# yozoyugen/HAKAI-fem

Measured on AMD Instinct MI355X. Metric: M element-updates/sec (hex8, 8 Gauss pts) at 1/2/4/8 MI355X; % HBM roofline, higher is better.
Workload: dtype f64

## Files before the change

### hakai-fem_amd/csrc/hakai_capi.cpp

```cpp
#include <hip/hip_runtime.h>

#include <algorithm>
#include <cmath>
#include <cstdarg>
#include <cstdio>
#include <cstdlib>
#include <cstring>
#include <map>
#include <memory>
#include <string>
#include <vector>

#include "../../include/hakai_hip.h"
#include "hakai_conn_plan.hpp"
#include "hakai_elem_history.hpp"
#include "hakai_history.hpp"
#include "hakai_internal.hpp"
#include "hakai_kernels.hpp"
#include "hakai_loads.hpp"
#include "hakai_mass_scale.hpp"
#include "hakai_stable_dt.hpp"

using hk::DevMat;

namespace {
thread_local std::string g_err;
}

namespace hkc {

int fail(int code, const char* fmt, ...) {
    char buf[1024];
    va_list ap;
    va_start(ap, fmt);
    vsnprintf(buf, sizeof buf, fmt, ap);
    va_end(ap);
    g_err = buf;
    return code;
}

int hip_fail(hipError_t e, const char* what) {
    return fail(HAKAI_ERR_DEVICE, "%s: %s", what, hipGetErrorString(e));
}

}

using hkc::DevBuf;
using hkc::fail;
using hkc::hip_fail;
using hkc::QSrc;

namespace hkc {

static void free_model(hakai_ctx* c) {
    contact_destroy(c);
    loads_destroy(c);
    for (DevBuf<double>* b : {&c->d_coord, &c->d_u[0], &c->d_u[1], &c->d_mass, &c->d_stress, &c->d_strain, &c->d_eqps,
                              &c->d_yield, &c->d_triax, &c->d_fe, &c->d_qbuf})
        b->free();
    for (DevBuf<int>* b : {&c->d_conn, &c->d_flag, &c->d_mat, &c->d_inc_ptr, &c->d_inc, &c->d_inc_row, &c->d_inc8,
                           &c->d_del_step})
        b->free();
    c->d_mats.free();
    c->d_conn_rec.free();
    c->conn_P = 0;
    own_free(c);
    c->model_ok = false;
    c->state_ok = false;
}

int build_devmat(const hakai_material_t& in, DevMat& o) {
    std::memset(&o, 0, sizeof o);
    const double young = in.young, poisson = in.poisson;
    const double d1 = (1.0 - poisson), d2 = poisson, d3 = (1.0 - 2.0 * poisson) / 2.0;
    const double cc = young / (1.0 + poisson) / (1.0 - 2.0 * poisson);
    o.Dn = cc * d1;
    o.Do = cc * d2;
    o.Ds = cc * d3;
    o.G = young / 2. / (1.0 + poisson);
    o.density = in.density;
    if (in.n_plastic < 0 || in.n_plastic > hk::kMaxPlastic)
        return fail(HAKAI_ERR_ARG, "material: %d plastic rows (max %d)", in.n_plastic, hk::kMaxPlastic);
    if (in.n_ductile < 0 || in.n_ductile > hk::kMaxDuctile)
        return fail(HAKAI_ERR_ARG, "material: %d ductile rows (max %d)", in.n_ductile, hk::kMaxDuctile);
    if (in.n_plastic == 1)
        return fail(HAKAI_ERR_MODEL,
                    "material: a single *Plastic row gives an empty Hd; the reference raises BoundsError "
                    "(v2/HAKAI_j.jl:1267)");
    o.npp = in.n_plastic;
    o.nd = in.n_ductile;
    o.yield0 = in.n_plastic > 0 ? in.plastic[0] : 0.0;
    for (int r = 0; r < in.n_plastic; ++r) o.pl_eps[r] = in.plastic[2 * r + 1];
    for (int r = 0; r + 1 < in.n_plastic; ++r)
        o.Hd[r] = (in.plastic[2 * (r + 1)] - in.plastic[2 * r]) / (in.plastic[2 * (r + 1) + 1] - in.plastic[2 * r + 1]);
    for (int r = 0; r < in.n_ductile; ++r) {
        o.du_eps[r] = in.ductile[3 * r + 0];
        o.du_tri[r] = in.ductile[3 * r + 1];
    }
    double lo = 0.0, hi = 0.0;
    for (int r = 0; r < in.n_ductile; ++r) {
        lo = r == 0 ? o.du_eps[r] : std::min(lo, o.du_eps[r]);
        hi = r == 0 ? o.du_eps[r] : std::max(hi, o.du_eps[r]);
    }
    o.du_floor = in.n_ductile > 0 ? lo - (std::fabs(hi) + std::fabs(lo)) * 0x1p-40 : 0.0;
    if (!(o.du_floor == o.du_floor)) o.du_floor = -HUGE_VAL;
    o.du_skip = o.du_floor > 0.0 ? o.du_floor - o.du_floor * 0x1p-40 : -HUGE_VAL;
    return 0;
}

void pusai_table(double out[192]) {
    static const double delta[8][3] = {{-1.0, -1.0, -1.0}, {1.0, -1.0, -1.0}, {1.0, 1.0, -1.0}, {-1.0, 1.0, -1.0},
                                       {-1.0, -1.0, 1.0},  {1.0, -1.0, 1.0},  {1.0, 1.0, 1.0},  {-1.0, 1.0, 1.0}};
    const double g = 1.0 / std::sqrt(3.0);
    for (int k = 0; k < 8; ++k) {
        const double gzai = (k & 4) ? g : -g, eta = (k & 2) ? g : -g, tueta = (k & 1) ? g : -g;
        for (int i = 0; i < 8; ++i) {
            out[24 * k + i] = 1.0 / 8.0 * delta[i][0] * (1.0 + eta * delta[i][1]) * (1.0 + tueta * delta[i][2]);
            out[24 * k + 8 + i] = 1.0 / 8.0 * delta[i][1] * (1.0 + gzai * delta[i][0]) * (1.0 + tueta * delta[i][2]);
            out[24 * k + 16 + i] = 1.0 / 8.0 * delta[i][2] * (1.0 + gzai * delta[i][0]) * (1.0 + eta * delta[i][1]);
        }
    }
}

hipStream_t ctx_stream(hakai_ctx* c) { return c->stream; }
int ctx_device(hakai_ctx* c) { return c->device; }

}

static void prof_harvest(hakai_ctx* c) {
    if (c->ev_pending.empty()) return;
    (void)hipEventSynchronize(c->ev_pending.back().b);
    for (auto& p : c->ev_pending) {
        float ms = 0.f;
        if (hipEventElapsedTime(&ms, p.a, p.b) == hipSuccess) {
            c->k_ms[p.kernel] += ms;
            c->k_n[p.kernel] += 1;
        }
        c->ev_pool.push_back(p.a);
        c->ev_pool.push_back(p.b);
    }
    c->ev_pending.clear();
}

static hipEvent_t prof_event(hakai_ctx* c) {
    if (c->ev_pool.empty()) {
        if (c->ev_pending.size() >= 2048) prof_harvest(c);
        if (c->ev_pool.empty()) {
            hipEvent_t e;
            (void)hipEventCreate(&e);
            return e;
        }
    }
    hipEvent_t e = c->ev_pool.back();
    c->ev_pool.pop_back();
    return e;
}

namespace hkc {
void prof_begin(hakai_ctx* c, int kernel, EventPair* p) {
    p->kernel = -1;
    if (!c->prof || !((c->prof_mask >> kernel) & 1u)) return;
    p->kernel = kernel;
    p->a = prof_event(c);
    p->b = prof_event(c);
    (void)hipEventRecord(p->a, c->stream);
}
void prof_end(hakai_ctx* c, EventPair* p) {
    if (!c->prof || p->kernel < 0) return;
    (void)hipEventRecord(p->b, c->stream);
    c->ev_pending.push_back(*p);
}
}


namespace hkc {

hk::ElemArgs elem_args(const hakai_ctx* c, int cur) {
    hk::ElemArgs ea;
    std::memset(&ea, 0, sizeof ea);
    ea.coord = c->d_coord;
    ea.u = c->d_u[cur];
    ea.u_pre = c->d_u[1 - cur];
    ea.conn = c->d_conn;
    ea.flag = c->d_flag;
    ea.mat = c->d_mat;
    ea.mat_stride = c->nmat == 1 ? 0u : 4u;
    ea.mats = c->d_mats;
    ea.stress = c->d_stress;
    ea.strain = c->d_strain;
    for (int q = 0; q < 6; ++q) {
        ea.sc[q] = c->d_stress + q * c->ld;
        ea.ec[q] = c->d_strain + q * c->ld;
    }
    ea.eqps = c->d_eqps;
    ea.yield = c->d_yield;
    ea.triax = c->d_triax;
    ea.fe = c->d_fe;
    ea.vol = nullptr;
    ea.nE = c->nE;
    ea.nEp = c->nEp;
    ea.ld = c->ld;
    ea.del_step = c->d_del_step;
    ea.step_i = 0;
    ea.any_plastic = c->any_plastic ? 1 : 0;
    ea.pipe_blocks = pipe_grid(c) > 0 ? c->pipe_blocks : 0;
    ea.gp_nt = c->gp_nt;
    ea.nmat = c->nmat;
    ea.exact = c->elem_exact;
    ea.pusai = c->d_pusai;
    ea.poison = c->d_poison;
    return ea;
}

hk::NodalArgs nodal_args(const hakai_ctx* c, double d_time) {
    hk::NodalArgs na;
    na.u = c->d_u[c->sv.cur];
    na.u_pre_out = c->d_u[1 - c->sv.cur];
    na.mass = c->d_mass;
    na.inc_ptr = c->d_inc_ptr;
    na.inc = c->d_inc;
    na.inc8 = c->d_inc8;
    na.fe = c->d_fe;
    na.qbuf = c->sv.q == QSrc::Buf ? c->d_qbuf : nullptr;
    na.fext = nullptr;
    na.nN = c->nN;
    na.dt = d_time;
    na.bc_of_node = nullptr;
    const OwnSums o = c->sv.q == QSrc::Own ? own_sums(c) : OwnSums{nullptr, nullptr, nullptr, nullptr};
    na.own_q = o.q;
    na.own_rp = o.rp;
    na.own_rows = o.rows;
    na.own_ridx = o.ridx;
    na.poison = c->d_poison;
    return na;
}

hk::BCArgs bc_args(const hakai_ctx* c, double t, double d_time) {
    hk::BCArgs ba;
    ba.dof = c->bc.d_dof;
    ba.grp = c->bc.d_grp;
    ba.val = c->bc.d_val;
    ba.n = c->bc.n;
    ba.amp_n = c->bc.d_amp_n;
    ba.amp_off = c->bc.d_amp_off;
    ba.amp_t = c->bc.d_amp_t;
    ba.amp_v = c->bc.d_amp_v;
    ba.out = c->d_u[1 - c->sv.cur];
    ba.ct = t * d_time;
    ba.t_rd = c->gr.trd;
    ba.dt = d_time;
    ba.poison = c->d_poison;
    return ba;
}

}

static int fe_download_qe(hakai_ctx* c, double* Qe) {
    HIPCHK(hipMemcpyAsync(Qe, c->d_fe, 24 * (size_t)c->nE * sizeof(double), hipMemcpyDeviceToHost, c->stream));
    HIPCHK(hipStreamSynchronize(c->stream));
    return 0;
}

static int fe_upload_qe(hakai_ctx* c, const double* Qe) {
    HIPCHK(hipMemcpyAsync(c->d_fe, Qe, 24 * (size_t)c->nE * sizeof(double), hipMemcpyHostToDevice, c->stream));
    HIPCHK(hipStreamSynchronize(c->stream));
    return 0;
}

static int fe_upload_incidence(hakai_ctx* c) {
    std::vector<int> inc(c->h_inc0.size());
    for (size_t j = 0; j < inc.size(); ++j) inc[j] = 24 * (c->h_inc0[j] >> 3) + 3 * (c->h_inc0[j] & 7);
    if (!inc.empty())
        HIPCHK(hipMemcpyAsync(c->d_inc, inc.data(), inc.size() * sizeof(int), hipMemcpyHostToDevice, c->stream));
    if (c->d_inc8) {
        std::vector<int> inc8(8 * (size_t)c->nN, (int)(24 * c->nEp));
        for (long long n = 0; n < c->nN; ++n)
            for (int j = c->h_ptr[n]; j < c->h_ptr[n + 1]; ++j) inc8[8 * n + (j - c->h_ptr[n])] = inc[j];
        HIPCHK(hipMemcpyAsync(c->d_inc8, inc8.data(), inc8.size() * sizeof(int), hipMemcpyHostToDevice, c->stream));
    }
    HIPCHK(hipStreamSynchronize(c->stream));
    return 0;
}

extern "C" {

int hakai_abi_version(void) { return HAKAI_ABI_VERSION; }
const char* hakai_last_error(void) { return g_err.c_str(); }

int hakai_device_count(int* n) {
    if (!n) return fail(HAKAI_ERR_ARG, "null");
    int cnt = 0;
    if (hipGetDeviceCount(&cnt) != hipSuccess) cnt = 0;
    *n = cnt;
    return 0;
}

int hakai_create(hakai_ctx** out, int device) {
    if (!out) return fail(HAKAI_ERR_ARG, "null ctx pointer");
    *out = nullptr;
    int cnt = 0;
    if (hipGetDeviceCount(&cnt) != hipSuccess || cnt <= 0)
        return fail(HAKAI_ERR_DEVICE, "no HIP device visible: the HAKAI MI355X path has no CPU fallback");
    if (device < 0 || device >= cnt) return fail(HAKAI_ERR_ARG, "device %d out of range (%d visible)", device, cnt);
    HIPCHK(hipSetDevice(device));
    hipDeviceProp_t prop;
    HIPCHK(hipGetDeviceProperties(&prop, device));
    if (std::strncmp(prop.gcnArchName, "gfx950", 6) != 0)
        return fail(HAKAI_ERR_DEVICE, "device %d is %s; libhakai_hip is built for gfx950 only", device,
                    prop.gcnArchName);
    struct Drop {
        void operator()(hakai_ctx* p) const {
            if (p->stream) (void)hipStreamDestroy(p->stream);
            delete p;
        }
    };
    std::unique_ptr<hakai_ctx, Drop> c(new hakai_ctx());
    c->device = device;
    if (const char* v = std::getenv("HAKAI_PIPE_BLOCKS")) c->pipe_blocks = std::atoi(v);
    if (const char* v = std::getenv("HAKAI_GRAPH")) {
        const int g = std::atoi(v);
        c->graph = (g >= 0 && g <= 1024 && !(g & 1)) ? g : 0;
    }
    hipError_t e = hipStreamCreateWithFlags(&c->stream, hipStreamNonBlocking);
    if (e != hipSuccess) return hip_fail(e, "hipStreamCreate");
    if (c->d_negjac.alloc(1) != hipSuccess || c->d_pusai.alloc(192) != hipSuccess ||
        c->d_poison.alloc(2) != hipSuccess || hipMemset(c->d_poison, 0, 2 * sizeof(int)) != hipSuccess)
        return fail(HAKAI_ERR_DEVICE, "hipMalloc for context bookkeeping failed");
    {
        double pus[192];
        hkc::pusai_table(pus);
        bool odd = true;
        for (int k = 0; k < 8; ++k)
            for (int i = 0; i < 8; ++i) {
                const double* p = pus + 24 * k;
                odd = odd && p[i] == -p[i ^ 1] && p[8 + i] == -p[8 + (i ^ 3)] && p[16 + i] == -p[16 + (i ^ 4)];
            }
        e = odd ? hipMemcpy(c->d_pusai, pus, sizeof pus, hipMemcpyHostToDevice) : hipErrorInvalidValue;
        if (e != hipSuccess) return hip_fail(e, "hipMemcpy (Pusai table)");
    }
    if (const char* v = std::getenv("HAKAI_ELEM_EXACT")) c->elem_exact = std::atoi(v) ? 1 : 0;
    if (const char* v = std::getenv("HAKAI_OWN_ASSEMBLY")) c->own.assembly = std::atoi(v) ? 1 : 0;
    *out = c.release();
    return 0;
}

int hakai_destroy(hakai_ctx* c) {
    if (!c) return 0;
    (void)hipSetDevice(c->device);
    (void)hipStreamSynchronize(c->stream);
    prof_harvest(c);
    hkc::graph_free(c);
    hkc::history_destroy(c);
    hkc::elem_history_destroy(c);
    hkc::stable_dt_destroy(c);
    hkc::mass_scale_destroy(c);
    hkc::comm_destroy(c);
    hkc::free_model(c);
    for (auto e : c->ev_pool) (void)hipEventDestroy(e);
    (void)hipStreamDestroy(c->stream);
    delete c;
    return 0;
}

int hakai_upload_model(hakai_ctx* c, int64_t nNode, const double* coordmat, int64_t nElement,
                       const int64_t* elementmat, const int64_t* element_material, int32_t nMat,
                       const hakai_material_t* mats, const double* diag_M) {
    if (c) hkc::graph_invalidate(c);
    if (!c) return fail(HAKAI_ERR_ARG, "null ctx");
    if (nNode <= 0 || nElement < 0 || !coordmat || (nElement > 0 && (!elementmat || !element_material)) || nMat <= 0 ||
        !mats || !diag_M)
        return fail(HAKAI_ERR_ARG, "upload_model: bad arguments");
    if (26 * (nElement + 32) + 8 >= (int64_t)INT32_MAX || nNode >= (int64_t)INT32_MAX)
        return fail(HAKAI_ERR_ARG, "upload_model: mesh too large for int32 indexing on one rank");
    if (192 * (nElement + 32) >= (int64_t)1 << 32)
        return fail(HAKAI_ERR_ARG, "upload_model: %lld elements exceed one context's 32-bit element-kernel offsets "
                    "(max %lld); split the mesh over ranks", (long long)nElement, (long long)(((int64_t)1 << 32) / 192 - 32));
    if (24 * (nNode + 1) >= (int64_t)1 << 32)
        return fail(HAKAI_ERR_ARG, "upload_model: %lld nodes exceed one context's 32-bit element-kernel offsets "
                    "(max %lld); split the mesh over ranks", (long long)nNode, (long long)(((int64_t)1 << 32) / 24 - 1));
    HIPCHK(hipSetDevice(c->device));
    (void)hipStreamSynchronize(c->stream);
    hkc::history_destroy(c);
    hkc::elem_history_destroy(c);
    hkc::stable_dt_destroy(c);
    hkc::mass_scale_destroy(c);
    hkc::free_model(c);
    c->bc = {};
    const long long nN = nNode, nE = nElement;
    const long long nEp = ((nE + 31) / 32) * 32;
    std::vector<int> conn((size_t)(8 * nEp), 0), mat((size_t)nEp, 0);
    for (long long e = 0; e < nE; ++e) {
        for (int i = 0; i < 8; ++i) {
            const int64_t n = elementmat[8 * e + i];
            if (n < 1 || n > nN) return fail(HAKAI_ERR_ARG, "elementmat[%d,%lld] = %lld out of 1..%lld", i + 1, e + 1, (long long)n, nN);
            conn[8 * e + i] = (int)(n - 1);
        }
        const int64_t m = element_material[e];
        if (m < 1 || m > nMat) return fail(HAKAI_ERR_ARG, "element_material[%lld] = %lld out of 1..%d", e + 1, (long long)m, nMat);
        mat[e] = (int)(m - 1);
    }
    std::vector<double> mass((size_t)nN);
    for (long long n = 0; n < nN; ++n) {
        const double m0 = diag_M[3 * n], m1 = diag_M[3 * n + 1], m2 = diag_M[3 * n + 2];
        if (!(m0 == m1 && m1 == m2))
            return fail(HAKAI_ERR_ARG, "diag_M: node %lld has different masses per dof", n + 1);
        mass[n] = m0;
    }
    c->h_mats.assign((size_t)nMat, DevMat());
    c->nmat = nMat;
    c->has_ductile = false;
    for (int i = 0; i < nMat; ++i) {
        int r = hkc::build_devmat(mats[i], c->h_mats[i]);
        if (r) return r;
    }
    c->any_plastic = false;
    for (long long e = 0; e < nE; ++e) {
        if (c->h_mats[mat[e]].nd > 0) c->has_ductile = true;
        if (c->h_mats[mat[e]].npp > 0) c->any_plastic = true;
    }
    std::vector<int> ptr((size_t)nN + 1, 0), inc((size_t)(8 * nE));
    for (long long j = 0; j < 8 * nE; ++j) ptr[conn[j] + 1]++;
    for (long long n = 0; n < nN; ++n) ptr[n + 1] += ptr[n];
    {
        std::vector<int> fill(ptr.begin(), ptr.end() - 1);
        for (long long j = 0; j < 8 * nE; ++j) inc[fill[conn[j]]++] = (int)j;
    }
    int maxinc = 0;
    for (long long n = 0; n < nN; ++n) maxinc = std::max(maxinc, ptr[n + 1] - ptr[n]);
    c->nN = nN;
    c->nE = nE;
    c->nEp = nEp;
    c->ld = 8 * nEp;
    const size_t ld = (size_t)c->ld;
    HIPCHK(c->d_coord.alloc(3 * (size_t)nN));
    HIPCHK(c->d_u[0].alloc(3 * (size_t)nN));
    HIPCHK(c->d_u[1].alloc(3 * (size_t)nN));
    HIPCHK(c->d_mass.alloc((size_t)nN));
    HIPCHK(c->d_conn.alloc(8 * (size_t)nEp));
    HIPCHK(c->d_flag.alloc((size_t)nEp));
    HIPCHK(c->d_mat.alloc((size_t)nEp));
    HIPCHK(c->d_del_step.alloc((size_t)nEp + 2));
    HIPCHK(c->d_mats.alloc((size_t)nMat));
    HIPCHK(c->d_stress.alloc(6 * ld));
    HIPCHK(c->d_strain.alloc(6 * ld));
    HIPCHK(c->d_eqps.alloc(ld));
    HIPCHK(c->d_yield.alloc(ld));
    HIPCHK(c->d_triax.alloc(ld));
    c->fe_len = 26 * nEp + 8;
    HIPCHK(c->d_fe.alloc((size_t)c->fe_len));
    HIPCHK(c->d_inc_ptr.alloc((size_t)nN + 1));
    HIPCHK(c->d_inc.alloc(8 * (size_t)nE));
    HIPCHK(c->d_inc_row.alloc(8 * (size_t)nE));
    HIPCHK(c->d_qbuf.alloc(3 * (size_t)nN));
    hipStream_t s = c->stream;
    HIPCHK(hipMemcpyAsync(c->d_coord, coordmat, 3 * nN * sizeof(double), hipMemcpyHostToDevice, s));
    HIPCHK(hipMemcpyAsync(c->d_mass, mass.data(), nN * sizeof(double), hipMemcpyHostToDevice, s));
    if (nE) {
        HIPCHK(hipMemcpyAsync(c->d_conn, conn.data(), 8 * nEp * sizeof(int), hipMemcpyHostToDevice, s));
        HIPCHK(hipMemcpyAsync(c->d_mat, mat.data(), nEp * sizeof(int), hipMemcpyHostToDevice, s));
        HIPCHK(hipMemcpyAsync(c->d_inc_row, inc.data(), 8 * nE * sizeof(int), hipMemcpyHostToDevice, s));
    }
    {
        hk::ConnPlan cp;
        if (nE && hk::conn_plan(conn.data(), nEp, cp)) {
            std::vector<unsigned> rp(cp.rec);
            rp.insert(rp.end(), cp.pat.begin(), cp.pat.end());
            HIPCHK(c->d_conn_rec.upload(rp, s));
            HIPCHK(hipStreamSynchronize(s));
            c->conn_P = cp.P;
            c->conn_bits = cp.base_bits;
            c->conn_bytes = cp.bytes;
        }
    }
    HIPCHK(hipMemcpyAsync(c->d_mats, c->h_mats.data(), nMat * sizeof(DevMat), hipMemcpyHostToDevice, s));
    HIPCHK(hipMemcpyAsync(c->d_inc_ptr, ptr.data(), (nN + 1) * sizeof(int), hipMemcpyHostToDevice, s));
    if (maxinc <= 8) HIPCHK(c->d_inc8.alloc(8 * (size_t)nN));
    HIPCHK(hipStreamSynchronize(s));
    c->max_inc = maxinc;
    c->h_ptr = ptr;
    c->h_inc0 = inc;
    {
        int r = fe_upload_incidence(c);
        if (r) return r;
    }
    c->h_coord.assign(coordmat, coordmat + 3 * nN);
    c->h_conn.assign(conn.begin(), conn.begin() + 8 * nE);
    c->h_mat.assign(mat.begin(), mat.begin() + nE);
    c->h_young.resize((size_t)nMat);
    for (int i = 0; i < nMat; ++i) c->h_young[i] = mats[i].young;
    c->h_poisson.resize((size_t)nMat);
    for (int i = 0; i < nMat; ++i) c->h_poisson[i] = mats[i].poisson;
    c->model_ok = true;
    c->state_ok = false;
    return hakai_reset_state(c, 0, nullptr, nullptr, 1.0);
}

int hakai_set_bc(hakai_ctx* c, const hakai_bc_t* bc) {
    if (c) hkc::graph_invalidate(c);
    if (!c || !bc) return fail(HAKAI_ERR_ARG, "null");
    if (!c->model_ok) return fail(HAKAI_ERR_STATE, "set_bc before upload_model");
    HIPCHK(hipSetDevice(c->device));
    (void)hipStreamSynchronize(c->stream);
    c->bc = {};
    const int G = bc->n_groups;
    if (G <= 0) return hkc::history_bc_changed(c);
    std::map<long long, std::pair<int, double>> last;
    for (int g = 0; g < G; ++g) {
        if (bc->amp_n[g] == 1)
            return fail(HAKAI_ERR_MODEL, "BC group %d: one-point amplitude, the reference raises BoundsError (:598)", g + 1);
        for (int64_t en = bc->entry_off[g]; en < bc->entry_off[g + 1]; ++en)
            for (int64_t d = bc->dof_off[en]; d < bc->dof_off[en + 1]; ++d) {
                const int64_t dof = bc->dofs[d];
                if (dof < 1 || dof > 3 * c->nN) return fail(HAKAI_ERR_ARG, "BC dof %lld out of range", (long long)dof);
                last[dof - 1] = std::make_pair(g, bc->entry_value[en]);
            }
    }
    std::vector<int> dof, grp;
    std::vector<double> val;
    for (auto& kv : last) {
        dof.push_back((int)kv.first);
        grp.push_back(kv.second.first);
        val.push_back(kv.second.second);
    }
    std::vector<int> amp_n(G), amp_off(G);
    long long n_amp = 0;
    for (int g = 0; g < G; ++g) {
        amp_n[g] = bc->amp_n[g];
        amp_off[g] = (int)bc->amp_off[g];
        n_amp = std::max<long long>(n_amp, bc->amp_off[g] + bc->amp_n[g]);
    }
    c->bc.n = (int)dof.size();
    HIPCHK(c->bc.d_dof.alloc(dof.size()));
    HIPCHK(c->bc.d_grp.alloc(grp.size()));
    HIPCHK(c->bc.d_val.alloc(val.size()));
    HIPCHK(c->bc.d_amp_n.alloc((size_t)G));
    HIPCHK(c->bc.d_amp_off.alloc((size_t)G));
    HIPCHK(c->bc.d_amp_t.alloc((size_t)n_amp));
    HIPCHK(c->bc.d_amp_v.alloc((size_t)n_amp));
    hipStream_t s = c->stream;
    if (!dof.empty()) {
        HIPCHK(hipMemcpyAsync(c->bc.d_dof, dof.data(), dof.size() * sizeof(int), hipMemcpyHostToDevice, s));
        HIPCHK(hipMemcpyAsync(c->bc.d_grp, grp.data(), grp.size() * sizeof(int), hipMemcpyHostToDevice, s));
        HIPCHK(hipMemcpyAsync(c->bc.d_val, val.data(), val.size() * sizeof(double), hipMemcpyHostToDevice, s));
    }
    HIPCHK(hipMemcpyAsync(c->bc.d_amp_n, amp_n.data(), G * sizeof(int), hipMemcpyHostToDevice, s));
    HIPCHK(hipMemcpyAsync(c->bc.d_amp_off, amp_off.data(), G * sizeof(int), hipMemcpyHostToDevice, s));
    if (n_amp) {
        HIPCHK(hipMemcpyAsync(c->bc.d_amp_t, bc->amp_time, n_amp * sizeof(double), hipMemcpyHostToDevice, s));
        HIPCHK(hipMemcpyAsync(c->bc.d_amp_v, bc->amp_value, n_amp * sizeof(double), hipMemcpyHostToDevice, s));
    }
    if (!dof.empty()) {
        std::vector<int> of((size_t)c->nN, -1);
        for (size_t i = dof.size(); i-- > 0;) of[(size_t)dof[i] / 3] = (int)i;
        HIPCHK(c->bc.d_of_node.alloc(of.size()));
        HIPCHK(hipMemcpyAsync(c->bc.d_of_node, of.data(), of.size() * sizeof(int), hipMemcpyHostToDevice, s));
    }
    HIPCHK(hipStreamSynchronize(s));
    return hkc::history_bc_changed(c);
}

int hakai_reset_state(hakai_ctx* c, int64_t n_ic, const int64_t* ic_dofs, const double* ic_values, double d_time) {
    if (c) hkc::graph_invalidate(c);
    if (!c) return fail(HAKAI_ERR_ARG, "null");
    if (!c->model_ok) return fail(HAKAI_ERR_STATE, "reset_state before upload_model");
    HIPCHK(hipSetDevice(c->device));
    hipStream_t s = c->stream;
    const size_t fn = 3 * (size_t)c->nN;
    c->sv.restart(false);
    HIPCHK(hipMemsetAsync(c->d_u[0], 0, fn * sizeof(double), s));
    HIPCHK(hipMemsetAsync(c->d_u[1], 0, fn * sizeof(double), s));
    HIPCHK(hipMemsetAsync(c->d_fe, 0, (size_t)c->fe_len * sizeof(double), s));
    HIPCHK(hipMemsetAsync(c->d_del_step, 0, ((size_t)c->nEp + 2) * sizeof(int), s));
    HIPCHK(hk::launch_reset_gp(c->d_stress, c->d_strain, c->d_eqps, c->d_yield, c->d_triax, c->d_flag, c->d_mat,
                               c->d_mats, c->nE, c->nEp, c->ld, s));
    c->h_velo0.assign(fn, 0.0);
    HIPCHK(hipMemsetAsync(c->d_poison, 0, 2 * sizeof(int), s));
    hkc::comm_reset(c);
    if (n_ic > 0) {
        if (!ic_dofs || !ic_values) return fail(HAKAI_ERR_ARG, "reset_state: null IC arrays");
        std::vector<double> dpre(fn, 0.0);
        for (int64_t j = 0; j < n_ic; ++j) {
            const int64_t d = ic_dofs[j];
            if (d < 1 || d > (int64_t)fn) return fail(HAKAI_ERR_ARG, "IC dof %lld out of range", (long long)d);
            dpre[d - 1] = -ic_values[j] * d_time;
            c->h_velo0[d - 1] = ic_values[j];
        }
        HIPCHK(hipMemcpyAsync(c->d_u[1 - c->sv.cur], dpre.data(), fn * sizeof(double), hipMemcpyHostToDevice, s));
        HIPCHK(hipStreamSynchronize(s));
    }
    c->state_ok = true;
    if (int r = hkc::contact_state_reset(c, c->h_velo0.data())) return r;
    if (int r = hkc::history_restart(c)) return r;
    if (int r = hkc::elem_history_restart(c)) return r;
    HIPCHK(hipStreamSynchronize(s));
    return 0;
}

int hakai_upload_state(hakai_ctx* c, const hakai_state_t* st) {
    if (c) hkc::graph_invalidate(c);
    if (!c || !st) return fail(HAKAI_ERR_ARG, "null");
    if (!c->model_ok) return fail(HAKAI_ERR_STATE, "upload_state before upload_model");
    HIPCHK(hipSetDevice(c->device));
    if (c->sv.q == QSrc::Own && !c->sv.fe_ok && !st->Q && !st->Qe) {
        bool dels = false;
        for (long long e = 0; st->element_flag && e < c->nE && !dels; ++e) dels = st->element_flag[e] == 0;
        if (dels || c->comm)
            return fail(HAKAI_ERR_STATE, "upload_state: the last element step's forces exist only as owner-computed "
                        "node sums (a contact overflow skipped the call's last step); upload Q (from "
                        "hakai_download_state) or Qe with this state");
        if (int r = hkc::own_materialize(c)) return r;
    }
    c->sv.restart(true);
    hipStream_t s = c->stream;
    const size_t fn = 3 * (size_t)c->nN, nGP = 8 * (size_t)c->nE;
    if (st->disp) HIPCHK(hipMemcpyAsync(c->d_u[c->sv.cur], st->disp, fn * sizeof(double), hipMemcpyHostToDevice, s));
    if (st->disp_pre)
        HIPCHK(hipMemcpyAsync(c->d_u[1 - c->sv.cur], st->disp_pre, fn * sizeof(double), hipMemcpyHostToDevice, s));
    if (st->velo) c->h_velo0.assign(st->velo, st->velo + fn);
    if (st->Q) {
        HIPCHK(hipMemcpyAsync(c->d_qbuf, st->Q, fn * sizeof(double), hipMemcpyHostToDevice, s));
        c->sv.q_uploaded();
    }
    if (st->integ_stress || st->integ_strain) {
        DevBuf<double> tmp;
        HIPCHK(tmp.alloc(6 * nGP));
        if (st->integ_stress) {
            HIPCHK(hipMemcpyAsync(tmp, st->integ_stress, 6 * nGP * sizeof(double), hipMemcpyHostToDevice, s));
            HIPCHK(hk::launch_aos_to_soa6(tmp, c->d_stress, (long long)nGP, c->ld, s));
        }
        if (st->integ_strain) {
            HIPCHK(hipMemcpyAsync(tmp, st->integ_strain, 6 * nGP * sizeof(double), hipMemcpyHostToDevice, s));
            HIPCHK(hk::launch_aos_to_soa6(tmp, c->d_strain, (long long)nGP, c->ld, s));
        }
        HIPCHK(hipStreamSynchronize(s));
    }
    if (st->integ_yield_stress)
        HIPCHK(hipMemcpyAsync(c->d_yield, st->integ_yield_stress, nGP * sizeof(double), hipMemcpyHostToDevice, s));
    if (st->integ_eq_plastic_strain)
        HIPCHK(hipMemcpyAsync(c->d_eqps, st->integ_eq_plastic_strain, nGP * sizeof(double), hipMemcpyHostToDevice, s));
    if (st->integ_triax_stress)
        HIPCHK(hipMemcpyAsync(c->d_triax, st->integ_triax_stress, nGP * sizeof(double), hipMemcpyHostToDevice, s));
    if (st->element_flag) {
        std::vector<int> f((size_t)c->nE);
        for (long long e = 0; e < c->nE; ++e) f[e] = st->element_flag[e] != 0 ? 1 : 0;
        HIPCHK(hipMemcpyAsync(c->d_flag, f.data(), c->nE * sizeof(int), hipMemcpyHostToDevice, s));
        std::vector<int> ds((size_t)c->nE);
        for (long long e = 0; e < c->nE; ++e) ds[e] = f[e] ? 0 : -1;
        HIPCHK(hipMemcpyAsync(c->d_del_step, ds.data(), c->nE * sizeof(int), hipMemcpyHostToDevice, s));
        HIPCHK(hipMemsetAsync(c->d_del_step + c->nEp, 0, 2 * sizeof(int), s));
        HIPCHK(hipStreamSynchronize(s));
        bool any = false;
        for (long long e = 0; e < c->nE; ++e) any |= !f[e];
        if (any && !st->Qe) {
            std::vector<double> qe(24 * (size_t)c->nE);
            int r = fe_download_qe(c, qe.data());
            if (r) return r;
            for (long long e = 0; e < c->nE; ++e)
                if (!f[e]) std::fill(qe.begin() + 24 * e, qe.begin() + 24 * (e + 1), 0.0);
            if ((r = fe_upload_qe(c, qe.data()))) return r;
        }
    }
    if (st->Qe) {
        int r = fe_upload_qe(c, st->Qe);
        if (r) return r;
    }
    HIPCHK(hipMemsetAsync(c->d_poison, 0, 2 * sizeof(int), s));
    HIPCHK(hipStreamSynchronize(s));
    hkc::comm_reset(c);
    c->state_ok = true;
    if (int r = hkc::history_restart(c)) return r;
    if (int r = hkc::elem_history_restart(c)) return r;
    if (c->contact) {
        if (int r = hkc::contact_state_reset(c, c->h_velo0.empty() ? nullptr : c->h_velo0.data())) return r;
        HIPCHK(hipStreamSynchronize(s));
    }
    return 0;
}

int hakai_download_state(hakai_ctx* c, hakai_state_t* st) {
    if (!c || !st) return fail(HAKAI_ERR_ARG, "null");
    if (!c->state_ok) return fail(HAKAI_ERR_STATE, "download_state without state");
    if (st->Qe && !c->sv.fe_ok)
        return fail(HAKAI_ERR_STATE, "download_state: Qe is not available after a call whose last steps a contact "
                    "overflow skipped (owner-computed assembly keeps node sums only); Q is -- or step once more");
    if (st->integ_triax_stress && !c->sv.triax_ok)
        return fail(HAKAI_ERR_STATE, "download_state: integ_triax_stress is not available after a call whose last "
                    "steps a contact overflow skipped (it is stored on a call's last step); step once more");
    HIPCHK(hipSetDevice(c->device));
    hipStream_t s = c->stream;
    const size_t fn = 3 * (size_t)c->nN, nGP = 8 * (size_t)c->nE;
    HIPCHK(hipStreamSynchronize(s));
    if (st->disp) HIPCHK(hipMemcpyAsync(st->disp, c->d_u[c->sv.cur], fn * sizeof(double), hipMemcpyDeviceToHost, s));
    if (st->disp_pre)
        HIPCHK(hipMemcpyAsync(st->disp_pre, c->d_u[1 - c->sv.cur], fn * sizeof(double), hipMemcpyDeviceToHost, s));
    if (st->velo) {
        if (c->sv.steps_done == 0) {
            std::memcpy(st->velo, c->h_velo0.data(), fn * sizeof(double));
        } else {
            std::vector<double> a(fn), b(fn);
            HIPCHK(hipMemcpyAsync(a.data(), c->d_u[c->sv.cur], fn * sizeof(double), hipMemcpyDeviceToHost, s));
            HIPCHK(hipMemcpyAsync(b.data(), c->d_u[1 - c->sv.cur], fn * sizeof(double), hipMemcpyDeviceToHost, s));
            HIPCHK(hipStreamSynchronize(s));
            for (size_t i = 0; i < fn; ++i) {
                const double dd = a[i] - b[i];
                st->velo[i] = dd / c->last_dt;
            }
        }
    }
    if (st->Q) {
        if (c->sv.q == QSrc::Buf) {
            HIPCHK(hipMemcpyAsync(st->Q, c->d_qbuf, fn * sizeof(double), hipMemcpyDeviceToHost, s));
        } else {
            DevBuf<double> tmp;
            HIPCHK(tmp.alloc(fn));
            if (c->sv.q == QSrc::Own) {
                const hkc::OwnSums o = hkc::own_sums(c);
                HIPCHK(hk::launch_own_q(o.q, o.rp, o.ridx, o.rows, tmp, c->nN, s));
            } else
                HIPCHK(hk::launch_gather_q(c->d_inc_ptr, c->d_inc, c->d_fe, tmp, c->nN, s));
            HIPCHK(hipMemcpyAsync(st->Q, tmp, fn * sizeof(double), hipMemcpyDeviceToHost, s));
            HIPCHK(hipStreamSynchronize(s));
        }
    }
    if (st->integ_stress || st->integ_strain) {
        DevBuf<double> tmp;
        HIPCHK(tmp.alloc(6 * nGP));
        if (st->integ_stress) {
            HIPCHK(hk::launch_soa_to_aos6(c->d_stress, tmp, (long long)nGP, c->ld, s));
            HIPCHK(hipMemcpyAsync(st->integ_stress, tmp, 6 * nGP * sizeof(double), hipMemcpyDeviceToHost, s));
            HIPCHK(hipStreamSynchronize(s));
        }
        if (st->integ_strain) {
            HIPCHK(hk::launch_soa_to_aos6(c->d_strain, tmp, (long long)nGP, c->ld, s));
            HIPCHK(hipMemcpyAsync(st->integ_strain, tmp, 6 * nGP * sizeof(double), hipMemcpyDeviceToHost, s));
            HIPCHK(hipStreamSynchronize(s));
        }
    }
    if (st->integ_yield_stress)
        HIPCHK(hipMemcpyAsync(st->integ_yield_stress, c->d_yield, nGP * sizeof(double), hipMemcpyDeviceToHost, s));
    if (st->integ_eq_plastic_strain)
        HIPCHK(hipMemcpyAsync(st->integ_eq_plastic_strain, c->d_eqps, nGP * sizeof(double), hipMemcpyDeviceToHost, s));
    if (st->integ_triax_stress)
        HIPCHK(hipMemcpyAsync(st->integ_triax_stress, c->d_triax, nGP * sizeof(double), hipMemcpyDeviceToHost, s));
    if (st->element_flag) {
        std::vector<int> f((size_t)c->nE);
        HIPCHK(hipMemcpyAsync(f.data(), c->d_flag, c->nE * sizeof(int), hipMemcpyDeviceToHost, s));
        HIPCHK(hipStreamSynchronize(s));
        for (long long e = 0; e < c->nE; ++e) st->element_flag[e] = (f[e] == 1) ? 1 : 0;
    }
    if (st->Qe) {
        int r = fe_download_qe(c, st->Qe);
        if (r) return r;
    }
    HIPCHK(hipStreamSynchronize(s));
    return 0;
}

int hakai_stat(hakai_ctx* c, const char* key, int64_t* value) {
    if (!c || !key || !value) return fail(HAKAI_ERR_ARG, "null");
    if (!std::strcmp(key, "graph_steps")) *value = c->graph_steps;
    else if (!std::strcmp(key, "device_buffers")) *value = hkc::g_dev_live.load();
    else if (!std::strcmp(key, "exchange_retries")) *value = c->exchange_retries;
    else if (!std::strncmp(key, "own_", 4) || !std::strncmp(key, "conn_", 5)) return hkc::own_stat(c, key, value);
    else return fail(HAKAI_ERR_ARG, "unknown stat '%s'", key);
    return 0;
}

int hakai_sync(hakai_ctx* c) {
    if (!c) return fail(HAKAI_ERR_ARG, "null");
    HIPCHK(hipSetDevice(c->device));
    HIPCHK(hipStreamSynchronize(c->stream));
    return 0;
}

int hakai_deleted(hakai_ctx* c, int64_t* n_deleted, int64_t* log, int64_t cap) {
    if (!c) return fail(HAKAI_ERR_ARG, "null");
    if (!c->model_ok) return fail(HAKAI_ERR_STATE, "deleted before upload_model");
    HIPCHK(hipSetDevice(c->device));
    std::vector<int> ds((size_t)c->nE);
    if (c->nE) HIPCHK(hipMemcpyAsync(ds.data(), c->d_del_step, c->nE * sizeof(int), hipMemcpyDeviceToHost, c->stream));
    HIPCHK(hipStreamSynchronize(c->stream));
    std::vector<std::pair<long long, long long>> v;
    for (long long e = 0; e < c->nE; ++e)
        if (ds[e] > 0) v.push_back(std::make_pair((long long)ds[e], e + 1 + c->elem_offset));
    std::sort(v.begin(), v.end());
    if (n_deleted) *n_deleted = (int64_t)v.size();
    if (log)
        for (long long i = 0; i < (long long)v.size() && i < cap; ++i) {
            log[2 * i] = v[i].first;
            log[2 * i + 1] = v[i].second;
        }
    return 0;
}

int hakai_set_tuning(hakai_ctx* c, const char* key, int64_t value) {
    if (c) hkc::graph_invalidate(c);
    if (!c || !key) return fail(HAKAI_ERR_ARG, "set_tuning: null");
    if (!std::strcmp(key, "elem_pipe_blocks")) {
        if (value < 0 || value > 65536) return fail(HAKAI_ERR_ARG, "elem_pipe_blocks out of range");
        c->pipe_blocks = (int)value;
        return 0;
    }
    if (!std::strcmp(key, "elem_gp_nt")) {
        if (value != 0 && value != 1) return fail(HAKAI_ERR_ARG, "elem_gp_nt must be 0 or 1");
        c->gp_nt = (int)value;
        return 0;
    }
    if (!std::strcmp(key, "fuse_bc")) {
        if (value < 0 || value > 2) return fail(HAKAI_ERR_ARG, "fuse_bc must be 0, 1 or 2 (any mesh size)");
        c->fuse_bc = (int)value;
        return 0;
    }
    if (!std::strcmp(key, "elem_pipe_min")) {
        if (value < 0 || value > 1024) return fail(HAKAI_ERR_ARG, "elem_pipe_min out of range");
        c->pipe_min = (int)value;
        return 0;
    }
    if (!std::strcmp(key, "elem_exact")) {
        if (value != 0 && value != 1) return fail(HAKAI_ERR_ARG, "elem_exact must be 0 or 1");
        if (c->elem_exact != (int)value)
            if (int r = hkc::own_tuning(c, key, value)) return r;
        c->elem_exact = (int)value;
        return 0;
    }
    if (!std::strcmp(key, "group_serial")) {
        if (value < 0 || value > 2) return fail(HAKAI_ERR_ARG, "group_serial must be 0, 1 or 2");
        c->group_serial = (int)value;
        return 0;
    }
    if (!std::strcmp(key, "nodal_padded")) {
        if (!value) {
            c->d_inc8.free();
            return 0;
        }
        return c->d_inc8 ? 0 : fail(HAKAI_ERR_STATE, "padded incidence table unavailable (>8 incidences)");
    }
    if (!std::strncmp(key, "own_", 4)) return hkc::own_tuning(c, key, value);
    if (!std::strcmp(key, "conn_templates")) {
        if (value != 0 && value != 1) return fail(HAKAI_ERR_ARG, "conn_templates must be 0 or 1");
        c->conn_templates = (int)value;
        return 0;
    }
    if (!std::strcmp(key, "graph")) {
        if (value < 0 || value > 1024 || (value & 1)) return fail(HAKAI_ERR_ARG, "graph must be 0 or an even step count <= 1024");
        c->graph = (int)value;
        return 0;
    }
    if (!std::strcmp(key, "history_one_block")) {
        if (value < -1 || value > 1) return fail(HAKAI_ERR_ARG, "history_one_block must be -1 (by size), 0 or 1");
        c->hist_one_block = (int)value;
        return 0;
    }
    if (!std::strcmp(key, "elem_history_one_block")) {
        if (value < -1 || value > 1) return fail(HAKAI_ERR_ARG, "elem_history_one_block must be -1 (by size), 0 or 1");
        c->ehist_one_block = (int)value;
        return 0;
    }
    if (!std::strncmp(key, "contact_", 8)) {
        HIPCHK(hipSetDevice(c->device));
        return hkc::contact_tuning(c, key, value);
    }
    return fail(HAKAI_ERR_ARG, "unknown tuning key '%s'", key);
}

int hakai_set_element_offset(hakai_ctx* c, int64_t element_offset) {
    if (c) hkc::graph_invalidate(c);
    if (!c || element_offset < 0) return fail(HAKAI_ERR_ARG, "set_element_offset: bad args");
    c->elem_offset = element_offset;
    return 0;
}

int hakai_negative_jacobians(hakai_ctx* c, int64_t* n) {
    if (!c || !n) return fail(HAKAI_ERR_ARG, "null");
    if (!c->state_ok) return fail(HAKAI_ERR_STATE, "negative_jacobians without state");
    HIPCHK(hipSetDevice(c->device));
    HIPCHK(hipMemsetAsync(c->d_negjac, 0, sizeof(unsigned long long), c->stream));
    HIPCHK(hk::launch_negjac(hkc::elem_args(c, c->sv.cur), c->d_negjac, c->stream));
    unsigned long long v = 0;
    HIPCHK(hipMemcpyAsync(&v, c->d_negjac, sizeof v, hipMemcpyDeviceToHost, c->stream));
    HIPCHK(hipStreamSynchronize(c->stream));
    *n = (int64_t)v;
    return 0;
}

int hakai_node_stress_strain(hakai_ctx* c, double* node_stress, double* node_strain, double* node_eqps,
                             double* node_mises, double* node_triax) {
    if (!c) return fail(HAKAI_ERR_ARG, "null");
    if (!c->state_ok) return fail(HAKAI_ERR_STATE, "node_stress_strain without state");
    HIPCHK(hipSetDevice(c->device));
    hipStream_t s = c->stream;
    const size_t nN = (size_t)c->nN;
    DevBuf<double> ns, nn, ne, nm, nt;
    HIPCHK(ns.alloc(6 * nN));
    HIPCHK(nn.alloc(6 * nN));
    HIPCHK(ne.alloc(nN));
    HIPCHK(nm.alloc(nN));
    HIPCHK(nt.alloc(nN));
    HIPCHK(hk::launch_node_average(c->d_inc_ptr, c->d_inc_row, c->d_stress, c->d_strain, c->d_eqps, c->d_triax, c->ld,
                                   c->nN, ns, nn, ne, nm, nt, s));
    if (node_stress) HIPCHK(hipMemcpyAsync(node_stress, ns, 6 * nN * sizeof(double), hipMemcpyDeviceToHost, s));
    if (node_strain) HIPCHK(hipMemcpyAsync(node_strain, nn, 6 * nN * sizeof(double), hipMemcpyDeviceToHost, s));
    if (node_eqps) HIPCHK(hipMemcpyAsync(node_eqps, ne, nN * sizeof(double), hipMemcpyDeviceToHost, s));
    if (node_mises) HIPCHK(hipMemcpyAsync(node_mises, nm, nN * sizeof(double), hipMemcpyDeviceToHost, s));
    if (node_triax) HIPCHK(hipMemcpyAsync(node_triax, nt, nN * sizeof(double), hipMemcpyDeviceToHost, s));
    HIPCHK(hipStreamSynchronize(s));
    return 0;
}

int hakai_profile_enable(hakai_ctx* c, int on) { return hakai_profile_mask(c, on ? (1u << HAKAI_K_COUNT) - 1 : 0u); }

int hakai_profile_mask(hakai_ctx* c, uint32_t mask) {
    if (c) hkc::graph_invalidate(c);
    if (!c) return fail(HAKAI_ERR_ARG, "null");
    if (!mask) prof_harvest(c);
    c->prof = mask != 0;
    c->prof_mask = mask;
    for (int k = 0; k < HAKAI_K_COUNT; ++k) {
        c->k_ms[k] = 0;
        c->k_n[k] = 0;
    }
    return 0;
}

int hakai_profile_read(hakai_ctx* c, int kernel, double* total_ms, int64_t* launches) {
    if (!c || kernel < 0 || kernel >= HAKAI_K_COUNT) return fail(HAKAI_ERR_ARG, "bad profile query");
    (void)hipSetDevice(c->device);
    prof_harvest(c);
    if (total_ms) *total_ms = c->k_ms[kernel];
    if (launches) *launches = c->k_n[kernel];
    return 0;
}

int hakai_stress_hexa(int device, int64_t nNode, int64_t nElement, double* Qe, double* integ_stress,
                      double* integ_strain, double* integ_yield_stress, double* integ_eq_plastic_strain,
                      const double* position, const double* d_disp, const int64_t* elementmat,
                      const int64_t* element_flag, int32_t integ_num, int32_t nMat, const hakai_material_t* mats,
                      const int64_t* element_material, double* elementVolume) {
    if (integ_num != 8) return fail(HAKAI_ERR_ARG, "integ_num must be 8 (v2/HAKAI_j.jl:177)");
    if (!Qe || !integ_stress || !integ_strain || !integ_yield_stress || !integ_eq_plastic_strain || !position ||
        !d_disp || !element_flag)
        return fail(HAKAI_ERR_ARG, "stress_hexa: null array");
    hakai_ctx* c = nullptr;
    int r = hakai_create(&c, device);
    if (r) return r;
    struct Guard {
        hakai_ctx* c;
        ~Guard() { hakai_destroy(c); }
    } guard{c};
    std::vector<double> ones(3 * (size_t)nNode, 1.0);
    r = hakai_upload_model(c, nNode, position, nElement, elementmat, element_material, nMat, mats, ones.data());
    if (r) return r;
    std::vector<double> zero(3 * (size_t)nNode, 0.0), mdu(3 * (size_t)nNode);
    for (size_t i = 0; i < mdu.size(); ++i) mdu[i] = -d_disp[i];
    hakai_state_t st;
    std::memset(&st, 0, sizeof st);
    st.disp = zero.data();
    st.disp_pre = mdu.data();
    st.integ_stress = integ_stress;
    st.integ_strain = integ_strain;
    st.integ_yield_stress = integ_yield_stress;
    st.integ_eq_plastic_strain = integ_eq_plastic_strain;
    st.element_flag = const_cast<int64_t*>(element_flag);
    r = hakai_upload_state(c, &st);
    if (r) return r;
    hipStream_t s = c->stream;
    DevBuf<double> d_vol;
    HIPCHK(d_vol.alloc((size_t)c->nEp));
    HIPCHK(hipMemsetAsync(c->d_fe, 0, 24 * (size_t)nElement * sizeof(double), s));
    hk::ElemArgs ea = hkc::elem_args(c, c->sv.cur);
    ea.vol = d_vol;
    ea.pipe_blocks = 0;
    HIPCHK(hk::launch_element(ea, false, false, s));
    std::vector<double> fe(24 * (size_t)nElement), vol((size_t)nElement);
    HIPCHK(hipMemcpyAsync(fe.data(), c->d_fe, fe.size() * sizeof(double), hipMemcpyDeviceToHost, s));
    HIPCHK(hipMemcpyAsync(vol.data(), d_vol, vol.size() * sizeof(double), hipMemcpyDeviceToHost, s));
    HIPCHK(hipStreamSynchronize(s));
    hakai_state_t out;
    std::memset(&out, 0, sizeof out);
    out.integ_stress = integ_stress;
    out.integ_strain = integ_strain;
    out.integ_yield_stress = integ_yield_stress;
    out.integ_eq_plastic_strain = integ_eq_plastic_strain;
    r = hakai_download_state(c, &out);
    if (r) return r;
    for (int64_t e = 0; e < nElement; ++e) {
        if (element_flag[e] == 0) continue;
        for (int j = 0; j < 24; ++j) Qe[24 * e + j] += fe[24 * e + j];
        if (elementVolume) elementVolume[e] = vol[e];
    }
    return 0;
}

int hakai_triax_stress(int device, int64_t nGP, const double* integ_stress, double* integ_triax_stress) {
    if (nGP < 0 || (nGP > 0 && (!integ_stress || !integ_triax_stress))) return fail(HAKAI_ERR_ARG, "triax: bad args");
    int cnt = 0;
    if (hipGetDeviceCount(&cnt) != hipSuccess || cnt <= device || device < 0)
        return fail(HAKAI_ERR_DEVICE, "no HIP device %d: no CPU fallback", device);
    HIPCHK(hipSetDevice(device));
    if (nGP == 0) return 0;
    DevBuf<double> st, tx;
    HIPCHK(st.alloc(6 * (size_t)nGP));
    HIPCHK(tx.alloc((size_t)nGP));
    HIPCHK(hipMemcpy(st, integ_stress, 6 * nGP * sizeof(double), hipMemcpyHostToDevice));
    HIPCHK(hk::launch_triax_aos(st, tx, nGP, 0));
    HIPCHK(hipMemcpy(integ_triax_stress, tx, nGP * sizeof(double), hipMemcpyDeviceToHost));
    return 0;
}

}

namespace hkc {
long long ctx_nN(hakai_ctx* c) { return c->nN; }
}
```

### hakai-fem_amd/csrc/hakai_elem_fused.hpp

```cpp
#pragma once
#include "hakai_elem_io.hpp"
#include "hakai_exact_math.hpp"

namespace hk {


template <bool DO_DELETE, bool STORE_TRIAX, bool ANY_PLASTIC, bool WITH_VOL, int NT = 0, bool OWN = false>
__device__ __forceinline__ void elem_step(const ElemArgs& a, const DevMat* __restrict__ mats, long long e, int k,
                                          double* nd8, const ElemIn& in, double* sfe = nullptr) {
    const DevMat* M = mats + in.mt;
    const bool active = in.fl == 1;
    const int npp = M->npp;
    const int nd = DO_DELETE ? M->nd : 0;
    double eqp = in.eqp, ys = in.ys;

    nd8[6 * k + 0] = in.x[0];
    nd8[6 * k + 1] = in.x[1];
    nd8[6 * k + 2] = in.x[2];
    nd8[6 * k + 3] = in.du[0];
    nd8[6 * k + 4] = in.du[1];
    nd8[6 * k + 5] = in.du[2];
    wave_lds_fence();

    const double g = 1.0 / __builtin_sqrt(3.0);
    const double hp = 1.0 + g, hm = 1.0 - g;
    int nodej[8];
#pragma unroll
    for (int j = 0; j < 8; ++j) nodej[j] = 6 * ref_of_sign(j ^ k);
#define HK_MG(j, b) ((((j) >> (b)) & 1) ? hm : hp)
#define HK_SG(j, b) ((((j) >> (b)) & 1) ? 1.0 : -1.0)
#define HK_D0(j) (HK_SG(j, 2) * (1.0 / 8.0 * HK_MG(j, 1) * HK_MG(j, 0)))
#define HK_D1(j) (HK_SG(j, 1) * (1.0 / 8.0 * HK_MG(j, 2) * HK_MG(j, 0)))
#define HK_D2(j) (HK_SG(j, 0) * (1.0 / 8.0 * HK_MG(j, 2) * HK_MG(j, 1)))
    double J[3][3] = {{0., 0., 0.}, {0., 0., 0.}, {0., 0., 0.}};
#pragma unroll
    for (int j = 0; j < 8; ++j) {
        const double* X = nd8 + nodej[j];
        const double X0 = X[0], X1 = X[1], X2 = X[2];
        const double p0 = HK_D0(j), p1 = HK_D1(j), p2 = HK_D2(j);
        J[0][0] += p0 * X0; J[0][1] += p0 * X1; J[0][2] += p0 * X2;
        J[1][0] += p1 * X0; J[1][1] += p1 * X1; J[1][2] += p1 * X2;
        J[2][0] += p2 * X0; J[2][1] += p2 * X1; J[2][2] += p2 * X2;
    }
    const double c11 = J[1][1] * J[2][2] - J[1][2] * J[2][1];
    const double c21 = J[1][2] * J[2][0] - J[1][0] * J[2][2];
    const double c31 = J[1][0] * J[2][1] - J[1][1] * J[2][0];
    const double dett = J[0][0] * c11 + J[0][1] * c21 + J[0][2] * c31;
    const double det = (__builtin_popcount(k) & 1) ? -dett : dett;
    const double rd = 1.0 / dett;
    const double i11 = c11 * rd, i21 = c21 * rd, i31 = c31 * rd;
    const double i12 = (J[0][2] * J[2][1] - J[0][1] * J[2][2]) * rd;
    const double i22 = (J[0][0] * J[2][2] - J[0][2] * J[2][0]) * rd;
    const double i32 = (J[0][1] * J[2][0] - J[0][0] * J[2][1]) * rd;
    const double i13 = (J[0][1] * J[1][2] - J[0][2] * J[1][1]) * rd;
    const double i23 = (J[0][2] * J[1][0] - J[0][0] * J[1][2]) * rd;
    const double i33 = (J[0][0] * J[1][1] - J[0][1] * J[1][0]) * rd;
    double P[8][3];
#pragma unroll
    for (int j = 0; j < 8; ++j) {
        const double p0 = HK_D0(j), p1 = HK_D1(j), p2 = HK_D2(j);
        P[j][0] = i11 * p0 + i12 * p1 + i13 * p2;
        P[j][1] = i21 * p0 + i22 * p1 + i23 * p2;
        P[j][2] = i31 * p0 + i32 * p1 + i33 * p2;
    }
#undef HK_D0
#undef HK_D1
#undef HK_D2
#undef HK_SG
#undef HK_MG

    const double V = allreduce8(fabs(det));
    double wbar[3];
    {
        double v[8][3];
#pragma unroll
        for (int j = 0; j < 8; ++j)
#pragma unroll
            for (int c = 0; c < 3; ++c) v[j][c] = det * P[j][c];
        reduce_scatter8_rel(v, wbar);
    }
    const double r3V = 1.0 / (3.0 * V);
    const double bb0 = wbar[0] * r3V, bb1 = wbar[1] * r3V, bb2 = wbar[2] * r3V;
    const double* dn = nd8 + nodej[0] + 3;
    const double sdot = allreduce8(bb0 * dn[0] + bb1 * dn[1] + bb2 * dn[2]);

    double Gm[3][3] = {{0., 0., 0.}, {0., 0., 0.}, {0., 0., 0.}};
#pragma unroll
    for (int j = 0; j < 8; ++j) {
        const double* D = nd8 + nodej[j] + 3;
        const double d0 = D[0], d1 = D[1], d2 = D[2];
#pragma unroll
        for (int c = 0; c < 3; ++c) {
            Gm[0][c] += d0 * P[j][c];
            Gm[1][c] += d1 * P[j][c];
            Gm[2][c] += d2 * P[j][c];
        }
    }
    constexpr double kThird = 1.0 / 3.0;
    const double vol = sdot - (Gm[0][0] + Gm[1][1] + Gm[2][2]) * kThird;
    double de[6];
    de[0] = Gm[0][0] + vol;
    de[1] = Gm[1][1] + vol;
    de[2] = Gm[2][2] + vol;
    de[3] = Gm[0][1] + Gm[1][0];
    de[4] = Gm[1][2] + Gm[2][1];
    de[5] = Gm[0][2] + Gm[2][0];

    const double Dn = M->Dn, Do = M->Do, Ds = M->Ds;
    double fin[6];
    fin[0] = in.sig[0] + (Dn * de[0] + Do * (de[1] + de[2]));
    fin[1] = in.sig[1] + (Dn * de[1] + Do * (de[0] + de[2]));
    fin[2] = in.sig[2] + (Dn * de[2] + Do * (de[0] + de[1]));
    fin[3] = in.sig[3] + Ds * de[3];
    fin[4] = in.sig[4] + Ds * de[4];
    fin[5] = in.sig[5] + Ds * de[5];
    const double mean = (fin[0] + fin[1] + fin[2]) * kThird;
    double dv0 = fin[0] - mean, dv1 = fin[1] - mean, dv2 = fin[2] - mean;
    const double q =
        sqrt(1.5 * (dv0 * dv0 + dv1 * dv1 + dv2 * dv2 + 2.0 * (fin[3] * fin[3] + fin[4] * fin[4] + fin[5] * fin[5])));
    double sc = 1.0;
    if (ANY_PLASTIC && npp > 0 && q > ys) {
        const int p = plastic_segment(M->pl_eps, npp, eqp);
        const double H = M->Hd[p];
        const double dep = (q - ys) / (3.0 * M->G + H);
        sc = (ys + H * dep) / q;
        dv0 *= sc;
        dv1 *= sc;
        dv2 *= sc;
        fin[0] = dv0 + mean;
        fin[1] = dv1 + mean;
        fin[2] = dv2 + mean;
        fin[3] *= sc;
        fin[4] *= sc;
        fin[5] *= sc;
        eqp += dep;
        ys += H * dep;
    }
    double eps[6];
#pragma unroll
    for (int c = 0; c < 6; ++c) eps[c] = in.eps[c] + de[c];

    const double oeq = q * sc;
    double tri = STORE_TRIAX ? ((oeq < 1e-10) ? 0.0 : mean / oeq) : 0.0;
    bool kill = false;
    if (DO_DELETE && nd > 0 && __builtin_amdgcn_ballot_w64(eqp >= M->du_skip) != 0) {
        const double v_e = allreduce8(eqp) * 0.125;
        if (!STORE_TRIAX) tri = (oeq < 1e-10) ? 0.0 : mean / oeq;
        const double t_e = allreduce8(tri) * 0.125;
        if (!(t_e < 0.0) && v_e >= M->du_floor)
            kill = active && v_e >= ductile_fr(M->du_eps, M->du_tri, nd, t_e);
    }

    double fk[3];
    {
        const double w00 = det * dv0, w11 = det * dv1, w22 = det * dv2;
        const double w01 = det * fin[3], w12 = det * fin[4], w02 = det * fin[5];
        double v[8][3];
#pragma unroll
        for (int i = 0; i < 8; ++i) {
            const double px = P[i][0], py = P[i][1], pz = P[i][2];
            v[i][0] = w00 * px + w01 * py + w02 * pz;
            v[i][1] = w01 * px + w11 * py + w12 * pz;
            v[i][2] = w02 * px + w12 * py + w22 * pz;
        }
        reduce_scatter8_rel(v, fk);
    }
    const double S = allreduce8(det * (3.0 * mean));
    fk[0] += S * bb0;
    fk[1] += S * bb1;
    fk[2] += S * bb2;
    if (WITH_VOL) a.vol[e] = V;
    elem_writeback<DO_DELETE, STORE_TRIAX, ANY_PLASTIC, NT, false, OWN>(a, e, k, in, active, kill, fk, fin, eps, eqp,
                                                                         ys, tri, sfe);
}

}
```

### hakai-fem_amd/csrc/hakai_element.hip

```cpp
#include <hip/hip_runtime.h>

#include <algorithm>
#include <type_traits>

#include "hakai_elem_exact.hpp"
#include "hakai_elem_fused.hpp"
#include "hakai_elem_io.hpp"
#include "hakai_kernels.hpp"
#include "hakai_own_pass.hpp"

namespace hk {

template <bool DO_DELETE, bool STORE_TRIAX, bool WITH_VOL, bool EXACT>
__global__ __launch_bounds__(kBlock, 2) void k_element(ElemArgs a) {
    __shared__ __attribute__((aligned(16))) double s_nd[kEPB * kLdsStride];
    __shared__ __attribute__((aligned(16))) double s_xb[EXACT ? kEPB * kXbStride : 1];
    __shared__ __attribute__((aligned(16))) double s_pus[EXACT ? 8 * kPusStride : 1];
    const long long vb = xcd_remap(blockIdx.x, gridDim.x);
    if (poisoned(a.poison)) return;
    graph_step(a);
    const int k = threadIdx.x & 7;
    const int grp = threadIdx.x >> 3;
    if (EXACT) {
        stage_pusai(a, s_pus);
        __syncthreads();
    }
    const long long e = vb * kEPB + grp;
    ElemIn in;
    load_stage_a<EXACT>(a, e, k, in);
    if (EXACT) {
        load_node_raw(a, in);
        load_gp<true>(a, e, k, in);
    } else {
        load_stage_b<true>(a, e, k, in);
    }
#ifdef HK_DIAG_PHASE
    PhaseClock pc;
#endif
    if (EXACT)
        elem_step_exact<DO_DELETE, STORE_TRIAX, true, WITH_VOL>(a, a.mats, e, k, s_nd + grp * kLdsStride,
                                                                s_xb + grp * kXbStride, s_pus, in, nullptr HK_PH_PASS);
    else
        elem_step<DO_DELETE, STORE_TRIAX, true, WITH_VOL>(a, a.mats, e, k, s_nd + grp * kLdsStride, in);
}

#ifdef HK_DIAG_WAVE
constexpr int kDiagWaves = 8192, kDiagWords = 8;
__device__ unsigned long long g_diag[kDiagWaves * kDiagWords];
#endif

template <bool DO_DELETE, bool STORE_TRIAX, bool ANY_PLASTIC, bool LDS_MATS, int NT, bool EXACT, int OS = 0,
          bool TPL = false, bool CT = false>
__global__ __launch_bounds__(kBlock, 2) void k_element_pipe(ElemArgs a) {
    constexpr bool OWN = OS > 0;
    constexpr int kOwnFe = OS * kEPB * kFeStride;
    __shared__ __attribute__((aligned(16))) double s_nd[kEPB * kLdsStride];
    __shared__ __attribute__((aligned(16))) double s_fe[OWN ? 2 * kOwnFe : 1];
    extern __shared__ __attribute__((aligned(16))) double s_dyn[];
    double* s_part = s_dyn;
    DevMat* s_mats = reinterpret_cast<DevMat*>(s_dyn + (OWN ? 3 * a.own_slots : 0));
    __shared__ __attribute__((aligned(16))) double s_xb[EXACT ? kEPB * kXbStride : 1];
    __shared__ __attribute__((aligned(16))) double s_pus[EXACT ? 8 * kPusStride : 1];
    if (poisoned(a.poison)) return;
    graph_step(a);
    const int k = threadIdx.x & 7;
    const int grp = threadIdx.x >> 3;
    if (LDS_MATS) {
        const int words = a.nmat * (int)(sizeof(DevMat) / sizeof(double));
        const double* src = reinterpret_cast<const double*>(a.mats);
        double* dst = reinterpret_cast<double*>(s_mats);
        for (int w = threadIdx.x; w < words; w += kBlock) dst[w] = src[w];
    }
    if (EXACT) stage_pusai(a, s_pus);
    if (LDS_MATS || EXACT) __syncthreads();
    const DevMat* mats = LDS_MATS ? s_mats : a.mats;
    double* nd8 = s_nd + grp * kLdsStride;
    double* xb = s_xb + (EXACT ? grp * kXbStride : 0);
    const long long nb = a.nEp / kEPB;
    long long first, stride, count;
    if (OWN) {
        first = a.own_bstart[blockIdx.x];
        stride = 1;
        count = a.own_bstart[blockIdx.x + 1] - first;
    } else if (gridDim.x % 8 != 0) {
        first = (long long)blockIdx.x * nb / gridDim.x;
        stride = 1;
        count = ((long long)blockIdx.x + 1) * nb / gridDim.x - first;
    } else {
        const long long x = blockIdx.x & 7, j = blockIdx.x >> 3, per = gridDim.x >> 3;
        const long long r0 = x * nb / 8, r1 = (x + 1) * nb / 8;
        first = r0 + j;
        stride = per;
        count = first < r1 ? (r1 - first + per - 1) / per : 0;
    }
    if (count <= 0) return;
    auto pos_of = [&](long long i) { return first + (i < count ? i : count - 1) * stride; };
    auto vb_of = [&](long long i) { return OWN ? (long long)a.own_seq[pos_of(i)] : pos_of(i); };
    auto elem_of = [&](long long i) { return vb_of(i) * kEPB + grp; };

#ifdef HK_DIAG_WAVE
    PassClock dg;
    const long long dg_t0 = clock64();
#endif
#ifdef HK_DIAG_PHASE
    PhaseClock pc;
#endif
    ElemIn cur, nxt;
    int4 ent_cur = {0, 0, 0, 0}, ent_nxt = {0, 0, 0, 0};
    load_stage_a<EXACT, CT>(a, elem_of(0), k, cur);
    load_stage_a<EXACT, CT>(a, elem_of(1), k, nxt);
    static_assert(!(CT && EXACT), "connectivity templates: fused kernel only");
    int rec_nn = 0;
    if (CT) {
        const int r0 = conn_rec(a, elem_of(0)), r1 = conn_rec(a, elem_of(1));
        cur.n = conn_node(a, r0, conn_off(a, r0, k));
        nxt.n = conn_node(a, r1, conn_off(a, r1, k));
        rec_nn = conn_rec(a, elem_of(2));
    }
    if (!EXACT) load_stage_b<ANY_PLASTIC, NT>(a, elem_of(0), k, cur);
    constexpr int S = OS > 0 ? OS : 1;
    auto sb_of = [&](long long i) { return pos_of((i < count ? i : count - 1) / S * S); };
    int4 hdr_cur = {0, 0, 0, 0}, hdr_nxt = {0, 0, 0, 0}, hdr_nn = {0, 0, 0, 0};
    if (OWN && TPL) {
        hdr_cur = own_hdr_load(a, sb_of(0));
        hdr_nxt = own_hdr_load(a, sb_of(1));
        ent_cur = own_load_tpl(a, hdr_cur);
    } else if (OWN) {
        ent_cur = own_load(a, sb_of(0));
    }
    for (long long i = 0; i < count; ++i) {
        ElemIn nn;
        load_stage_a<EXACT, CT>(a, elem_of(i + 2), k, nn);
        int off = 0;
        if (CT) {
            nn.n = rec_nn;
            rec_nn = conn_rec(a, elem_of(i + 3));
            off = conn_off(a, nn.n, k);
        }
        if (OWN && TPL) hdr_nn = own_hdr_load(a, sb_of(i + 2));
        if (!EXACT) load_stage_b<ANY_PLASTIC, NT>(a, elem_of(i + 1), k, nxt);
        if (OWN) ent_nxt = TPL ? own_load_tpl(a, hdr_nxt) : own_load(a, sb_of(i + 1));
        double* sfe = s_fe + ((i / S) & 1) * kOwnFe + (i % S) * (kEPB * kFeStride);
        if (EXACT) {
#ifdef HK_DIAG_PHASE
            pc.last = clock64();
#endif
            load_node_raw(a, cur);
            load_gp<ANY_PLASTIC, NT>(a, elem_of(i), k, cur);
            HK_PH(pc, 0);
            elem_step_exact<DO_DELETE, STORE_TRIAX, ANY_PLASTIC, false, NT, OWN>(a, mats, elem_of(i), k, nd8, xb, s_pus,
                                                                                 cur, sfe HK_PH_PASS);
        }
        else
            elem_step<DO_DELETE, STORE_TRIAX, ANY_PLASTIC, false, NT, OWN>(a, mats, elem_of(i), k, nd8, cur, sfe);
        if (OWN) {
            if ((i + 1) % S == 0 || i + 1 == count)
                own_pass<TPL>(a, ent_cur, hdr_cur, sb_of(i), s_fe + ((i / S) & 1) * kOwnFe, s_part HK_DIAG_PASS);
            ent_cur = ent_nxt;
            if (TPL) {
                hdr_cur = hdr_nxt;
                hdr_nxt = hdr_nn;
            }
        }
        if (CT) nn.n = conn_node(a, nn.n, off);
        cur = nxt;
        nxt = nn;
    }
#ifdef HK_DIAG_WAVE
    const long long dg_t1 = clock64();
    const unsigned gw = blockIdx.x * (kBlock / 64) + threadIdx.x / 64;
    if ((threadIdx.x & 63) == 0 && gw < (unsigned)kDiagWaves) {
        unsigned long long* d = g_diag + (size_t)kDiagWords * gw;
        atomicAdd(d + 0, (unsigned long long)(dg_t1 - dg_t0));
        atomicAdd(d + 1, (unsigned long long)dg.bar);
        atomicAdd(d + 2, (unsigned long long)dg.pass);
        atomicAdd(d + 3, (unsigned long long)dg.n);
        atomicAdd(d + 4, (unsigned long long)count);
        atomicAdd(d + 5, 1ull);
        atomicExch(d + 6, (unsigned long long)__builtin_amdgcn_s_getreg((31 << 11) | 4));
#ifdef HK_DIAG_PHASE
        unsigned long long* q = g_diag + (size_t)kDiagWords * (kDiagWaves / 2 + gw);
        for (int j = 0; j < 8; ++j) atomicAdd(q + j, (unsigned long long)pc.t[j]);
#endif
    }
#endif
}

#ifdef HK_DIAG_WAVE
extern "C" int hk_diag_reset() {
    void* p = nullptr;
    if (hipGetSymbolAddress(&p, HIP_SYMBOL(g_diag)) != hipSuccess) return -1;
    return hipMemset(p, 0, sizeof(g_diag)) == hipSuccess ? 0 : -1;
}
extern "C" int hk_diag_read(unsigned long long* out, int n) {
    if (hipDeviceSynchronize() != hipSuccess) return -1;
    return hipMemcpyFromSymbol(out, HIP_SYMBOL(g_diag), sizeof(unsigned long long) * (size_t)std::min(n, kDiagWaves * kDiagWords)) == hipSuccess ? 0 : -1;
}
#endif

template <class T, T... Vs>
struct Sel {
    T v;
};
static Sel<bool, false, true> sel(bool v) { return {v}; }
template <int... Vs>
static Sel<int, Vs...> sel(int v) {
    return {v};
}
template <class F>
static void with_consts(F&& f) {
    f();
}
template <class F, class T, T... Vs, class... Rest>
static void with_consts(F&& f, Sel<T, Vs...> s, Rest... rest) {
    (void)((s.v == Vs &&
            (with_consts([&](auto... cs) { f(std::integral_constant<T, Vs>{}, cs...); }, rest...), true)) ||
           ...);
}

constexpr bool pipe_exists(bool lds_mats, bool exact, int os, bool tpl, bool ct) {
    return (os > 0 ? lds_mats : !tpl) && (!ct || (!exact && tpl));
}

static void launch_pipe(const ElemArgs& a, bool do_delete, bool store_triax, unsigned grid, hipStream_t s) {
    const int os = a.own == 1 || a.own == 2 ? a.own : 0;
    const bool lds = os > 0 || a.nmat <= kMaxLdsMats;
    const bool tpl = os > 0 && a.own_hdr;
    const bool ct = !a.exact && tpl && a.conn_rec;
    const size_t dyn = (os > 0 ? 24 * (size_t)a.own_slots : 0) + (lds ? sizeof(DevMat) * (size_t)a.nmat : 0);
    with_consts(
        [&](auto DD, auto ST, auto AP, auto LDS, auto NT, auto EX, auto OS, auto TPL, auto CT) {
            if constexpr (pipe_exists(LDS(), EX(), OS(), TPL(), CT()))
                hipLaunchKernelGGL((k_element_pipe<DD(), ST(), AP(), LDS(), NT(), EX(), OS(), TPL(), CT()>), dim3(grid),
                                   dim3(kBlock), dyn, s, a);
        },
        sel(do_delete), sel(store_triax), sel(a.any_plastic != 0), sel(lds), sel<0, 3>(a.gp_nt ? 3 : 0),
        sel(a.exact != 0), sel<0, 1, 2>(os), sel(tpl), sel(ct));
}

static void launch_batch(const ElemArgs& a, bool do_delete, bool store_triax, unsigned grid, hipStream_t s) {
    const bool with_vol = a.vol != nullptr;
    with_consts(
        [&](auto DD, auto ST, auto VOL, auto EX) {
            if constexpr (!VOL() || (!DD() && !ST()))
                hipLaunchKernelGGL((k_element<DD(), ST(), VOL(), EX()>), dim3(grid), dim3(kBlock), 0, s, a);
        },
        sel(!with_vol && do_delete), sel(!with_vol && store_triax), sel(with_vol), sel(a.exact != 0));
}

hipError_t launch_element(const ElemArgs& a, bool do_delete, bool store_triax, hipStream_t s) {
    if (a.nE <= 0) return hipSuccess;
    if (a.exact && !a.pusai) return hipErrorInvalidValue;
    const long long nb = a.nEp / kEPB;
    if (nb <= 0) return hipSuccess;
    if (a.own) {
        if (a.own > 2 || a.vol || a.pipe_blocks <= 0 || a.nmat > kMaxLdsMats || !(a.own_off || a.own_hdr) || !a.own_list ||
            !a.own_seq || !a.own_bstart || !a.own_q || !a.own_dump || a.own_slots < 1 ||
            a.own_slots > own_slot_cap(a.exact != 0, a.own, a.nmat))
            return hipErrorInvalidValue;
        if (a.own_grid <= 0 || a.own_grid > nb) return hipErrorInvalidValue;
        if (a.conn_rec && (a.conn_bits < 0 || a.conn_bits > 31)) return hipErrorInvalidValue;
        launch_pipe(a, do_delete, store_triax, (unsigned)a.own_grid, s);
    } else if (a.pipe_blocks > 0 && !a.vol) {
        launch_pipe(a, do_delete, store_triax, (unsigned)std::min<long long>(nb, a.pipe_blocks), s);
    } else {
        launch_batch(a, do_delete, store_triax, (unsigned)nb, s);
    }
    return hipGetLastError();
}

__global__ void k_negjac(ElemArgs a, unsigned long long* count) {
    const long long t = (long long)blockIdx.x * blockDim.x + threadIdx.x;
    if (t >= 8 * a.nE) return;
    const long long e = t >> 3;
    const int k = t & 7;
    if (a.flag[e] != 1) return;
    const double g = 1.0 / __builtin_sqrt(3.0);
    const double gz = (k & 4) ? g : -g, et = (k & 2) ? g : -g, tu = (k & 1) ? g : -g;
    double J[3][3] = {{0., 0., 0.}, {0., 0., 0.}, {0., 0., 0.}};
    for (int i = 0; i < 8; ++i) {
        const long long n = a.conn[8 * e + i];
        const double p0 = 0.125 * kSx[i] * (1.0 + et * kSy[i]) * (1.0 + tu * kSz[i]);
        const double p1 = 0.125 * kSy[i] * (1.0 + gz * kSx[i]) * (1.0 + tu * kSz[i]);
        const double p2 = 0.125 * kSz[i] * (1.0 + gz * kSx[i]) * (1.0 + et * kSy[i]);
        for (int c = 0; c < 3; ++c) {
            const double X = a.coord[3 * n + c] + a.u[3 * n + c];
            J[0][c] += p0 * X;
            J[1][c] += p1 * X;
            J[2][c] += p2 * X;
        }
    }
    const double det = J[0][0] * (J[1][1] * J[2][2] - J[1][2] * J[2][1]) +
                       J[0][1] * (J[1][2] * J[2][0] - J[1][0] * J[2][2]) +
                       J[0][2] * (J[1][0] * J[2][1] - J[1][1] * J[2][0]);
    if (det < 0.0) atomicAdd(count, 1ull);
}

hipError_t launch_negjac(const ElemArgs& a, unsigned long long* count, hipStream_t s) {
    if (a.nE <= 0) return hipSuccess;
    hipLaunchKernelGGL(k_negjac, dim3((unsigned)((8 * a.nE + 255) / 256)), dim3(256), 0, s, a, count);
    return hipGetLastError();
}

}
```

### hakai-fem_amd/csrc/hakai_internal.hpp

```cpp
#pragma once
#include <hip/hip_runtime.h>

#include <string>
#include <vector>

#include "../../include/hakai_hip.h"
#include "hakai_device.hpp"
#include "hakai_devmem.hpp"
#include "hakai_kernels.hpp"
#include "hakai_own.hpp"
#include "hakai_step_view.hpp"

namespace hkc {
struct Comm;
struct Contact;
struct History;
struct ElemHistory;
struct StableDt;
struct Loads;
struct MassScale;
int fail(int code, const char* fmt, ...);
int hip_fail(hipError_t e, const char* what);
}

struct EventPair {
    hipEvent_t a, b;
    int kernel;
};


constexpr long long kFuseBcMaxNodes = 1 << 18;

struct hakai_ctx {
    int device = 0;
    hipStream_t stream = nullptr;
    long long nN = 0, nE = 0, nEp = 0, ld = 0;
    hkc::DevBuf<double> d_coord;
    hkc::DevBuf<double> d_u[2];
    hkc::StepView sv;
    hkc::DevBuf<double> d_mass;
    hkc::DevBuf<int> d_conn;
    hkc::DevBuf<unsigned> d_conn_rec;
    int conn_P = 0, conn_bits = 0;
    long long conn_bytes = 0;
    int conn_templates = 1;
    hkc::DevBuf<int> d_flag;
    hkc::DevBuf<int> d_mat;
    hkc::DevBuf<hk::DevMat> d_mats;
    std::vector<hk::DevMat> h_mats;
    bool has_ductile = false;
    hkc::DevBuf<double> d_stress, d_strain, d_eqps, d_yield, d_triax, d_fe;
    hkc::DevBuf<int> d_inc_ptr;
    hkc::DevBuf<int> d_inc;
    hkc::DevBuf<int> d_inc_row;
    hkc::DevBuf<int> d_inc8;
    long long fe_len = 0;
    int max_inc = 0;
    std::vector<int> h_ptr, h_inc0;
    int pipe_blocks = 512;
    int pipe_min = 2;
    int gp_nt = 1;
    int elem_exact = 0;
    int group_serial = 0;
    hkc::DevBuf<double> d_pusai;
    int nmat = 0;
    long long elem_offset = 0;
    struct BcTables {
        int n = 0;
        hkc::DevBuf<int> d_dof, d_grp;
        hkc::DevBuf<double> d_val;
        hkc::DevBuf<int> d_amp_n, d_amp_off;
        hkc::DevBuf<double> d_amp_t, d_amp_v;
        hkc::DevBuf<int> d_of_node;
    } bc;
    int fuse_bc = 1;
    hkc::DevBuf<double> d_qbuf;
    std::vector<double> h_velo0;
    double last_dt = 0.0;
    hkc::DevBuf<int> d_del_step;
    hkc::DevBuf<unsigned long long> d_negjac;
    hkc::DevBuf<int> d_poison;
    long long poison_step = -1;
    long long exchange_retries = 0;
    bool any_plastic = false;
    bool model_ok = false;
    bool state_ok = false;
    std::vector<double> h_coord;
    std::vector<int> h_conn;
    std::vector<int> h_mat;
    std::vector<double> h_young;
    double* d_fext = nullptr;
    hkc::Contact* contact = nullptr;
    bool prof = false;
    uint32_t prof_mask = 0;
    std::vector<hipEvent_t> ev_pool;
    std::vector<EventPair> ev_pending;
    double k_ms[HAKAI_K_COUNT] = {0, 0, 0, 0};
    long long k_n[HAKAI_K_COUNT] = {0, 0, 0, 0};
    hkc::DevBuf<double> d_tstep;
    struct StepGraphs {
        const double* trd = nullptr;
        hipGraphExec_t exec[2][2] = {{nullptr, nullptr}, {nullptr, nullptr}};
        double dt[2][2] = {{0.0, 0.0}, {0.0, 0.0}};
        long long epoch[2][2] = {{-1, -1}, {-1, -1}};
        int len[2][2] = {{0, 0}, {0, 0}};
    } gr;
    long long epoch = 0;
    long long tdev_next = -1;
    int graph = 16;
    long long graph_steps = 0;
    hkc::Own own;
    hkc::Comm* comm = nullptr;
    hkc::History* hist = nullptr;
    int hist_one_block = -1;
    hkc::ElemHistory* ehist = nullptr;
    int ehist_one_block = -1;
    hkc::StableDt* sdt = nullptr;
    std::vector<double> h_poisson;
    hkc::MassScale* msc = nullptr;
    hkc::Loads* loads = nullptr;
    double* d_ftot = nullptr;
};


namespace hkc {
inline const double* step_fext(const hakai_ctx* c) {
    return c->d_ftot ? c->d_ftot : (c->contact ? c->d_fext : nullptr);
}
inline long long pipe_grid(const hakai_ctx* c) {
    const long long nb = c->nEp / hk::kEPB;
    const bool pipe = nb >= (long long)c->pipe_min * c->pipe_blocks && c->pipe_blocks > 0;
    return pipe ? (nb < c->pipe_blocks ? nb : c->pipe_blocks) : 0;
}
hk::ElemArgs elem_args(const hakai_ctx* c, int cur);
hk::NodalArgs nodal_args(const hakai_ctx* c, double d_time);
hk::BCArgs bc_args(const hakai_ctx* c, double t, double d_time);
void prof_begin(hakai_ctx* c, int kernel, EventPair* p);
void prof_end(hakai_ctx* c, EventPair* p);
void comm_destroy(hakai_ctx* c);
int comm_reset(hakai_ctx* c);
void comm_pending_get(const hakai_ctx* c, bool* pending, int* par);
void comm_rollback(hakai_ctx* c, bool had_good, long long last_good, bool pending, int par);
int comm_pre_nodal(hakai_ctx* c);
struct CommFix {
    bool ran = false;
    int n_up = 0, nslot = 0;
    const double* up_sendP = nullptr;
    const double* up_recvC = nullptr;
};
int comm_post_nodal(hakai_ctx* c, double d_time, CommFix* fix = nullptr);
int comm_post_element(hakai_ctx* c, long long step);
bool comm_is_local(const hakai_ctx* c);
const std::vector<int>* comm_dn_nodes(const hakai_ctx* c);
const std::vector<int>* comm_up_nodes(const hakai_ctx* c);
bool comm_iface_set(const hakai_ctx* c);
int comm_rank(const hakai_ctx* c);
int comm_size(const hakai_ctx* c);
constexpr int kMaxLocalGather = 64;
struct LocalGather {
    const char* src[kMaxLocalGather];
    long long bytes[kMaxLocalGather];
    long long off[kMaxLocalGather];
};
int gather_local(hakai_ctx* c, const LocalGather& g, int n, void* dst);
int comm_allgather_raw(hakai_ctx* c, const void* send, void* recv, size_t bytes);
int comm_allgatherv_raw(hakai_ctx* c, const void* send, void* recv, const size_t* bytes, const size_t* off);
int comm_allreduce_min_u64(hakai_ctx* c, const void* send, void* recv, size_t count);
bool comm_is_rccl(const hakai_ctx* c);
hakai_ctx* comm_peer_ctx(hakai_ctx* c, int q);
void contact_destroy(hakai_ctx* c);
int contact_state_reset(hakai_ctx* c, const double* velo0_host);
int contact_step(hakai_ctx* c, double t, double d_time);
int contact_phase(hakai_ctx* c, int part, double t, double d_time);
int contact_step_b(hakai_ctx* c);
bool contact_multi(const hakai_ctx* c);
int contact_post_step(hakai_ctx* c);
int contact_check(hakai_ctx* c);
void contact_after_overflow(hakai_ctx* c, long long steps_since_reset);
bool contact_exchange_retry(hakai_ctx* c);
void graph_invalidate(hakai_ctx* c);
void graph_free(hakai_ctx* c);
bool contact_graph_ok(const hakai_ctx* c, double t);
void contact_graph_advance(hakai_ctx* c, double t_last);
int contact_tuning(hakai_ctx* c, const char* key, long long value);
}
```

### hakai-fem_amd/csrc/hakai_kernels.hpp

```cpp
#pragma once
#include <hip/hip_runtime.h>
#include <stdint.h>

#include "hakai_device.hpp"
#include "hakai_own_entry.hpp"

namespace hk {

constexpr int kBlock = 256;
constexpr int kEPB = kBlock / 8;

struct ElemArgs {
    const double* coord;
    const double* u;
    const double* u_pre;
    const int* conn;
    const unsigned* conn_rec;
    int conn_bits;
    int* flag;
    const int* mat;
    unsigned mat_stride;
    const DevMat* mats;
    double* stress;
    double* strain;
    double* sc[6];
    double* ec[6];
    double* eqps;
    double* yield;
    double* triax;
    double* fe;
    double* vol;
    long long nE;
    long long nEp;
    long long ld;
    int* del_step;
    int step_i;
    const double* t_rd;
    double* t_wr;
    int any_plastic;
    int pipe_blocks;
    int nmat;
    int gp_nt;
    int exact;
    const double* pusai;
    const int* poison;
    int own;
    int own_grid;
    const int* own_seq;
    const int* own_bstart;
    const int* own_off;
    const int4* own_list;
    const int4* own_hdr;
    int own_nop;
    int own_slots;
    double* own_q;
    double* own_rows;
    double* own_dump;
};

struct BCArgs {
    const int* dof;
    const int* grp;
    const double* val;
    int n;
    const int* amp_n;
    const int* amp_off;
    const double* amp_t;
    const double* amp_v;
    double* out;
    double ct;
    const double* t_rd;
    double dt;
    const int* poison;
};

struct NodalArgs {
    const double* u;
    double* u_pre_out;
    const double* mass;
    const int* inc_ptr;
    const int* inc;
    const int* inc8;
    const double* fe;
    const double* qbuf;
    const double* fext;
    long long nN;
    double dt;
    const int* bc_of_node;
    BCArgs bc;
    const int* poison;
    const double* own_q;
    const int* own_rp;
    const int* own_ridx;
    const double* own_rows;
};


inline int own_slot_cap(bool exact, int batches_per_pass, int nmat) {
    const int stat = 12800 + 6400 * batches_per_pass * 2 + (exact ? 20608 : 0) + 64;
    const int left = 81920 - 256 - stat - nmat * (int)sizeof(DevMat);
    return left < 24 ? 0 : (left / 24 > kOwnSlotsMax ? kOwnSlotsMax : left / 24);
}

hipError_t launch_element(const ElemArgs& a, bool do_delete, bool store_triax, hipStream_t s);
hipError_t launch_negjac(const ElemArgs& a, unsigned long long* count, hipStream_t s);
hipError_t launch_nodal(const NodalArgs& a, hipStream_t s);
hipError_t launch_bc(const BCArgs& a, hipStream_t s);
hipError_t launch_set_step(double* slot, double t_prev, hipStream_t s);
hipError_t launch_hold(int rounds, hipStream_t s);

hipError_t launch_gather_q(const int* inc_ptr, const int* inc, const double* fe, double* Q, long long nN,
                           hipStream_t s);
hipError_t launch_own_q(const double* own_q, const int* rp, const int* ridx, const double* rows, double* Q,
                        long long nN, hipStream_t s);
hipError_t launch_aos_to_soa6(const double* aos, double* soa, long long nGP, long long ld, hipStream_t s);
hipError_t launch_soa_to_aos6(const double* soa, double* aos, long long nGP, long long ld, hipStream_t s);
hipError_t launch_reset_gp(double* stress, double* strain, double* eqps, double* yield, double* triax, int* flag,
                           const int* mat, const DevMat* mats, long long nE, long long nEp, long long ld, hipStream_t s);
hipError_t launch_triax_aos(const double* stress_aos, double* triax, long long nGP, hipStream_t s);
hipError_t launch_node_average(const int* inc_ptr, const int* inc, const double* stress, const double* strain,
                               const double* eqps, const double* triax, long long ld, long long nN,
                               double* node_stress, double* node_strain, double* node_eqps, double* node_mises,
                               double* node_triax, hipStream_t s);

}
```

### hakai-fem_amd/csrc/hakai_nodal.hip

```cpp
#include <hip/hip_runtime.h>

#include "hakai_kernels.hpp"

namespace hk {

__device__ __forceinline__ double bc_value(const BCArgs& a, int i) {
#pragma clang fp contract(off)
    const int g = a.grp[i];
    const double ct = a.t_rd ? (*a.t_rd + 1.0) * a.dt : a.ct;
    double amp = 1.0;
    const int na = a.amp_n[g];
    if (na > 0) {
        const double* at = a.amp_t + a.amp_off[g];
        const double* av = a.amp_v + a.amp_off[g];
        int ti = 0;
        for (int j = 0; j < na - 1; ++j)
            if (ct >= at[j] && ct <= at[j + 1]) {
                ti = j;
                break;
            }
        amp = av[ti] + (av[ti + 1] - av[ti]) * (ct - at[ti]) / (at[ti + 1] - at[ti]);
    }
    return a.val[i] * amp;
}

struct NodeIn {
    double m, uc[3], up[3], f[3];
};

template <bool FEXT>
__device__ __forceinline__ void nodal_load(const NodalArgs& a, long long n, NodeIn& in) {
    in.m = a.mass[n];
#pragma unroll
    for (int c = 0; c < 3; ++c) {
        in.uc[c] = a.u[3 * n + c];
        in.up[c] = a.u_pre_out[3 * n + c];
        in.f[c] = FEXT ? a.fext[3 * n + c] : 0.0;
    }
}

template <bool BCF>
__device__ __forceinline__ void nodal_update(const NodalArgs& a, long long n, const NodeIn& in, double Q0, double Q1,
                                             double Q2) {
#pragma clang fp contract(off)
    const double m = in.m;
    const double dt = a.dt;
    const double dC = 0.0 * m;
    const double mdt2 = m / (dt * dt);
    const double inv = 1.0 / (mdt2 + dC / 2.0 / dt);
    const double Q[3] = {Q0, Q1, Q2};
    const int b0 = BCF ? a.bc_of_node[n] : -1;
#pragma unroll
    for (int c = 0; c < 3; ++c) {
        const double up = in.up[c];
        double v = inv * (in.f[c] - Q[c] + mdt2 * (2.0 * in.uc[c] - up) + dC / 2.0 / dt * up);
        if (BCF) {
            const long long dc = 3 * n + c;
            for (int j = b0; j >= 0 && j < a.bc.n && a.bc.dof[j] <= dc; ++j)
                if (a.bc.dof[j] == dc) v = bc_value(a.bc, j);
        }
        a.u_pre_out[3 * n + c] = v;
    }
}

template <int MODE, bool FEXT, bool BCF>
__global__ __launch_bounds__(kBlock) void k_nodal(NodalArgs a) {
#pragma clang fp contract(off)
    if (poisoned(a.poison)) return;
    const unsigned lb = xcd_remap_rev(blockIdx.x, gridDim.x);
    const long long n = (long long)lb * kBlock + threadIdx.x;
    if (n >= a.nN) return;
    NodeIn in;
    nodal_load<FEXT>(a, n, in);
    double Q0 = 0.0, Q1 = 0.0, Q2 = 0.0;
    if (MODE == 2) {
        Q0 = a.qbuf[3 * n + 0];
        Q1 = a.qbuf[3 * n + 1];
        Q2 = a.qbuf[3 * n + 2];
    } else if (MODE == 3) {
        Q0 = a.own_q[3 * n + 0];
        Q1 = a.own_q[3 * n + 1];
        Q2 = a.own_q[3 * n + 2];
        const int j0 = a.own_rp[n], j1 = a.own_rp[n + 1];
        for (int j = j0; j < j1; ++j) {
            const long long r = a.own_ridx[j];
            Q0 += a.own_rows[3 * r + 0];
            Q1 += a.own_rows[3 * r + 1];
            Q2 += a.own_rows[3 * r + 2];
        }
    } else if (MODE == 0) {
        const int4 lo = reinterpret_cast<const int4*>(a.inc8)[2 * n];
        const int4 hi = reinterpret_cast<const int4*>(a.inc8)[2 * n + 1];
        const int idx[8] = {lo.x, lo.y, lo.z, lo.w, hi.x, hi.y, hi.z, hi.w};
        double f[8][3];
#pragma unroll
        for (int j = 0; j < 8; ++j) {
            const double* p = a.fe + idx[j];
            f[j][0] = p[0];
            f[j][1] = p[1];
            f[j][2] = p[2];
        }
#pragma unroll
        for (int j = 0; j < 8; ++j) {
            Q0 += f[j][0];
            Q1 += f[j][1];
            Q2 += f[j][2];
        }
    } else {
        const int j0 = a.inc_ptr[n], j1 = a.inc_ptr[n + 1];
        for (int j = j0; j < j1; ++j) {
            const double* f = a.fe + a.inc[j];
            Q0 += f[0];
            Q1 += f[1];
            Q2 += f[2];
        }
    }
    nodal_update<BCF>(a, n, in, Q0, Q1, Q2);
}

template <bool FEXT, bool BCF>
static void launch_nodal_m(const NodalArgs& a, unsigned grid, hipStream_t s) {
    if (a.qbuf)
        hipLaunchKernelGGL((k_nodal<2, FEXT, BCF>), dim3(grid), dim3(kBlock), 0, s, a);
    else if (a.own_q)
        hipLaunchKernelGGL((k_nodal<3, FEXT, BCF>), dim3(grid), dim3(kBlock), 0, s, a);
    else if (a.inc8)
        hipLaunchKernelGGL((k_nodal<0, FEXT, BCF>), dim3(grid), dim3(kBlock), 0, s, a);
    else
        hipLaunchKernelGGL((k_nodal<1, FEXT, BCF>), dim3(grid), dim3(kBlock), 0, s, a);
}

hipError_t launch_nodal(const NodalArgs& a, hipStream_t s) {
    if (a.nN <= 0) return hipSuccess;
    const unsigned grid = (unsigned)((a.nN + kBlock - 1) / kBlock);
    if (a.bc_of_node) {
        if (a.fext)
            launch_nodal_m<true, true>(a, grid, s);
        else
            launch_nodal_m<false, true>(a, grid, s);
    } else {
        if (a.fext)
            launch_nodal_m<true, false>(a, grid, s);
        else
            launch_nodal_m<false, false>(a, grid, s);
    }
    return hipGetLastError();
}

__global__ __launch_bounds__(kBlock) void k_bc(BCArgs a) {
    if (poisoned(a.poison)) return;
    const int i = blockIdx.x * kBlock + threadIdx.x;
    if (i >= a.n) return;
    a.out[a.dof[i]] = bc_value(a, i);
}

hipError_t launch_bc(const BCArgs& a, hipStream_t s) {
    if (a.n <= 0) return hipSuccess;
    hipLaunchKernelGGL(k_bc, dim3((a.n + kBlock - 1) / kBlock), dim3(kBlock), 0, s, a);
    return hipGetLastError();
}

__global__ void k_set_step(double* slot, double t_prev) {
    if (threadIdx.x == 0) *slot = t_prev;
}

__global__ void k_hold(int rounds) {
    for (int i = 0; i < rounds; ++i) __builtin_amdgcn_s_sleep(127);
}

hipError_t launch_hold(int rounds, hipStream_t s) {
    hipLaunchKernelGGL(k_hold, dim3(1), dim3(64), 0, s, rounds);
    return hipGetLastError();
}

hipError_t launch_set_step(double* slot, double t_prev, hipStream_t s) {
    hipLaunchKernelGGL(k_set_step, dim3(1), dim3(64), 0, s, slot, t_prev);
    return hipGetLastError();
}

__global__ void k_gather_q(const int* __restrict__ ptr, const int* __restrict__ inc, const double* __restrict__ fe,
                           double* Q, long long nN) {
#pragma clang fp contract(off)
    const long long n = (long long)blockIdx.x * blockDim.x + threadIdx.x;
    if (n >= nN) return;
    double q0 = 0.0, q1 = 0.0, q2 = 0.0;
    for (int j = ptr[n]; j < ptr[n + 1]; ++j) {
        const double* f = fe + inc[j];
        q0 += f[0];
        q1 += f[1];
        q2 += f[2];
    }
    Q[3 * n + 0] = q0;
    Q[3 * n + 1] = q1;
    Q[3 * n + 2] = q2;
}

hipError_t launch_gather_q(const int* inc_ptr, const int* inc, const double* fe, double* Q, long long nN,
                           hipStream_t s) {
    if (nN <= 0) return hipSuccess;
    hipLaunchKernelGGL(k_gather_q, dim3((unsigned)((nN + 255) / 256)), dim3(256), 0, s, inc_ptr, inc, fe, Q, nN);
    return hipGetLastError();
}

__global__ void k_own_q(const double* __restrict__ own_q, const int* __restrict__ rp, const int* __restrict__ ridx,
                        const double* __restrict__ rows, double* Q, long long nN) {
#pragma clang fp contract(off)
    const long long n = (long long)blockIdx.x * blockDim.x + threadIdx.x;
    if (n >= nN) return;
    double q0 = own_q[3 * n + 0], q1 = own_q[3 * n + 1], q2 = own_q[3 * n + 2];
    for (int j = rp[n]; j < rp[n + 1]; ++j) {
        const long long r = ridx[j];
        q0 += rows[3 * r + 0];
        q1 += rows[3 * r + 1];
        q2 += rows[3 * r + 2];
    }
    Q[3 * n + 0] = q0;
    Q[3 * n + 1] = q1;
    Q[3 * n + 2] = q2;
}

hipError_t launch_own_q(const double* own_q, const int* rp, const int* ridx, const double* rows, double* Q,
                        long long nN, hipStream_t s) {
    if (nN <= 0) return hipSuccess;
    hipLaunchKernelGGL(k_own_q, dim3((unsigned)((nN + 255) / 256)), dim3(256), 0, s, own_q, rp, ridx, rows, Q, nN);
    return hipGetLastError();
}

}
```

### hakai-fem_amd/csrc/hakai_own.cpp

```cpp
#include "hakai_own.hpp"

#include <algorithm>
#include <cstring>
#include <vector>

#include "hakai_internal.hpp"
#include "hakai_own_plan.hpp"

namespace hkc {

static bool own_live(const hakai_ctx* c) { return c->sv.q == QSrc::Own; }

void own_free(hakai_ctx* c) {
    c->own.l = Own::Lists();
    c->own.for_g0 = -1;
    c->sv.own_dropped();
}

void own_invalidate(hakai_ctx* c) {
    c->own.l.built_g = -1;
    c->own.for_g0 = -1;
    c->sv.own_dropped();
}

OwnSums own_sums(const hakai_ctx* c) {
    const Own::Lists& l = c->own.l;
    return {l.d_q, l.d_rp, l.d_ridx, l.d_rows};
}

static bool own_upload(hakai_ctx* c, const hk::OwnSched& sc, const hk::OwnPlan& pl) {
    own_free(c);
    Own::Lists& l = c->own.l;
    const long long nN = c->nN, G = (long long)sc.bstart.size() - 1;
    std::vector<int> bst(sc.bstart.begin(), sc.bstart.end());
    hipStream_t s = c->stream;
    if ((pl.tpl ? l.d_hdr.upload(pl.hdr, s) || l.d_list.upload(pl.tlist, s)
                : l.d_off.upload(pl.off, s) || l.d_list.upload(pl.list, s)) ||
        l.d_seq.upload(sc.seq, s) || l.d_bstart.upload(bst, s) || l.d_rp.upload(pl.rp, s) || l.d_ridx.upload(pl.ridx, s) ||
        l.d_q.alloc(3 * (size_t)nN) || l.d_rows.alloc(3 * (size_t)std::max(pl.rows, 1LL)) ||
        l.d_dump.alloc(8 * (size_t)G) ||
        hipMemsetAsync(l.d_q, 0, 3 * (size_t)nN * sizeof(double), s) ||
        hipStreamSynchronize(s)) {
        own_free(c);
        return false;
    }
    l.nop = (int)(pl.tpl ? pl.stored : pl.ne);
    l.slots = pl.tpl ? pl.P : pl.max_slots;
    l.stored = pl.tpl ? pl.stored : pl.ne;
    l.templates = pl.tpl ? pl.templates : 0;
    l.rows = pl.rows;
    l.entries = pl.ne;
    l.built_g = G;
    l.s = pl.S;
    l.round2 = pl.round2;
    l.banded = sc.banded ? 1 : 0;
    return true;
}

int own_materialize(hakai_ctx* c) {
    if (!own_live(c)) return 0;
    if (c->comm)
        return fail(HAKAI_ERR_STATE, "owner-computed assembly cannot be switched off or rebuilt on a multi-GPU rank "
                    "mid-run: upload or reset the state first");
    const OwnSums o = own_sums(c);
    HIPCHK(hk::launch_own_q(o.q, o.rp, o.ridx, o.rows, c->d_qbuf, c->nN, c->stream));
    c->sv.q_uploaded();
    return 0;
}

static long long own_g0(const hakai_ctx* c) {
    if (!c->own.assembly || c->nmat > hk::kMaxLdsMats || c->nE <= 0) return 0;
    return pipe_grid(c);
}

bool own_wanted(const hakai_ctx* c) {
    const Own& o = c->own;
    const long long G0 = own_g0(c);
    if (G0 <= 0 || o.for_g0 != G0 || o.l.built_g <= 0) return false;
    return !(c->elem_exact && o.l.round2 > 0 && o.assembly == 1 && !(c->comm && own_live(c)));
}

bool own_prepare(hakai_ctx* c) {
    const long long G0 = own_g0(c);
    if (G0 > 0 && c->own.for_g0 != G0) {
        if (own_live(c) && own_materialize(c)) return false;
        const hk::OwnInput in{c->nE, c->nN, c->nEp, c->h_conn, c->h_ptr, c->h_inc0, c->max_inc,
                              c->own.band_rows, c->own.pass_batches, comm_dn_nodes(c),
                              {hk::own_slot_cap(c->elem_exact != 0, 1, c->nmat),
                               hk::own_slot_cap(c->elem_exact != 0, 2, c->nmat)},
                              c->own.templates};
        hk::OwnSched sc;
        hk::OwnPlan pl;
        if (!(hk::own_choose(in, G0, sc, pl) && own_upload(c, sc, pl))) {
            own_free(c);
            c->own.l.built_g = -2;
        }
        c->own.for_g0 = G0;
    }
    return own_wanted(c);
}

static bool conn_in_use(const hakai_ctx* c) {
    return c->conn_templates && c->conn_P > 0 && !c->elem_exact && own_wanted(c) && c->own.l.d_hdr.get();
}

void own_elem_args(const hakai_ctx* c, hk::ElemArgs& ea) {
    const Own::Lists& l = c->own.l;
    ea.own = l.s;
    ea.own_grid = (int)l.built_g;
    ea.own_seq = l.d_seq;
    ea.own_bstart = l.d_bstart;
    ea.own_off = l.d_off;
    ea.own_list = reinterpret_cast<const int4*>(l.d_list.get());
    ea.own_hdr = reinterpret_cast<const int4*>(l.d_hdr.get());
    ea.own_nop = l.nop;
    ea.own_slots = l.slots;
    ea.own_q = l.d_q;
    ea.own_rows = l.d_rows;
    ea.own_dump = l.d_dump;
    if (conn_in_use(c)) {
        ea.conn_rec = c->d_conn_rec;
        ea.conn_bits = c->conn_bits;
    }
}

int own_tuning(hakai_ctx* c, const char* key, long long value) {
    Own& o = c->own;
    if (!std::strcmp(key, "own_assembly")) {
        if (value < 0 || value > 2) return fail(HAKAI_ERR_ARG, "own_assembly must be 0, 1 or 2");
        o.assembly = (int)value;
        return 0;
    }
    if (!std::strcmp(key, "own_pass_batches")) {
        if (value < 0 || value > 2) return fail(HAKAI_ERR_ARG, "own_pass_batches must be 0, 1 or 2");
        if (o.pass_batches != (int)value) o.for_g0 = -1;
        o.pass_batches = (int)value;
        return 0;
    }
    if (!std::strcmp(key, "own_templates")) {
        if (value < 0 || value > 1) return fail(HAKAI_ERR_ARG, "own_templates must be 0 or 1");
        if (o.templates != (int)value) o.for_g0 = -1;
        o.templates = (int)value;
        return 0;
    }
    if (!std::strcmp(key, "own_band_rows")) {
        if (value < 0 || value > 4096) return fail(HAKAI_ERR_ARG, "own_band_rows must be in [0, 4096]");
        if (o.band_rows != (int)value) o.for_g0 = -1;
        o.band_rows = (int)value;
        return 0;
    }
    if (!std::strcmp(key, "elem_exact")) {
        if (o.for_g0 == -1) return 0;
        if (!(c->comm && own_live(c))) {
            o.for_g0 = -1;
        } else if (o.l.built_g > 0 && o.l.slots > hk::own_slot_cap(value != 0, o.l.s, c->nmat)) {
            return fail(HAKAI_ERR_STATE, "elem_exact: the owner-assembly lists of this multi-GPU rank need %d LDS "
                        "slots, more than the %s kernel has; switch between calls after hakai_upload_state / "
                        "hakai_reset_state", o.l.slots, value ? "reference-order" : "fused");
        }
        return 0;
    }
    return fail(HAKAI_ERR_ARG, "unknown tuning key '%s'", key);
}

int own_stat(const hakai_ctx* c, const char* key, int64_t* value) {
    const Own::Lists& l = c->own.l;
    const bool built = l.built_g > 0;
    if (!std::strcmp(key, "own_steps")) *value = c->own.steps;
    else if (!std::strcmp(key, "own_rows")) *value = built ? l.rows : -1;
    else if (!std::strcmp(key, "own_entries")) *value = built ? l.entries : -1;
    else if (!std::strcmp(key, "own_entries_stored")) *value = built ? l.stored : -1;
    else if (!std::strcmp(key, "own_templates")) *value = built ? l.templates : 0;
    else if (!std::strcmp(key, "own_superbatch")) *value = built ? l.s : 0;
    else if (!std::strcmp(key, "own_round2")) *value = built ? l.round2 : 0;
    else if (!std::strcmp(key, "own_slots")) *value = built ? l.slots : 0;
    else if (!std::strcmp(key, "own_banded")) *value = built ? l.banded : 0;
    else if (!std::strcmp(key, "own_grid")) *value = built ? l.built_g : 0;
    else if (!std::strcmp(key, "conn_patterns")) *value = conn_in_use(c) ? c->conn_P : 0;
    else if (!std::strcmp(key, "conn_bytes")) *value = conn_in_use(c) ? c->conn_bytes : 32 * c->nEp;
    else return fail(HAKAI_ERR_ARG, "unknown stat '%s'", key);
    return 0;
}

}
```

### hakai-fem_amd/csrc/hakai_own.hpp

```cpp
#pragma once
#include "hakai_devmem.hpp"
#include "hakai_kernels.hpp"

struct hakai_ctx;

namespace hkc {

struct Own {
    int assembly = 1;
    int band_rows = 0;
    int pass_batches = 0;
    int templates = 1;
    long long for_g0 = -1;
    long long steps = 0;
    struct Lists {
        long long built_g = -1;
        DevBuf<int> d_off;
        DevBuf<int> d_seq;
        DevBuf<int> d_bstart;
        int banded = 0;
        long long round2 = 0;
        DevBuf<int> d_list;
        DevBuf<int> d_hdr;
        long long stored = 0;
        long long templates = 0;
        int nop = 0;
        int slots = 0;
        DevBuf<double> d_q;
        DevBuf<int> d_rp;
        DevBuf<double> d_rows;
        DevBuf<int> d_ridx;
        DevBuf<double> d_dump;
        long long rows = 0, entries = 0;
        int s = 2;
    } l;
};

struct OwnSums {
    const double* q;
    const int* rp;
    const int* ridx;
    const double* rows;
};
OwnSums own_sums(const hakai_ctx* c);

void own_free(hakai_ctx* c);
void own_invalidate(hakai_ctx* c);
bool own_prepare(hakai_ctx* c);
bool own_wanted(const hakai_ctx* c);
int own_materialize(hakai_ctx* c);
void own_elem_args(const hakai_ctx* c, hk::ElemArgs& ea);
int own_tuning(hakai_ctx* c, const char* key, long long value);
int own_stat(const hakai_ctx* c, const char* key, int64_t* value);

}
```

### hakai-fem_amd/csrc/hakai_own_entry.hpp

```cpp
#pragma once

#if defined(__HIPCC__) || defined(__CUDACC__)
#define HK_HD __host__ __device__ __forceinline__
#else
#define HK_HD static inline
#endif

namespace hk {

enum { kOwnInit = 1, kOwnFin = 2, kOwnExp = 4, kOwnNop = 8 };
constexpr int kOwnExpRows = 4;
constexpr int kOwnSlotsMax = 2048;
constexpr int kOwnRound2 = 1 << 27;

HK_HD constexpr int own_pack_y(int slot, int flags, int n, int lane7) {
    return (int)(((unsigned)slot & 1023u) | (unsigned)flags << 10 | (unsigned)n << 14 | (unsigned)lane7 << 18 |
                 ((unsigned)slot & 1024u) << 18);
}
static_assert((own_pack_y(kOwnSlotsMax - 1, 15, 15, 511) & kOwnRound2) == 0, "kOwnRound2 overlaps a packed field");

HK_HD void own_pack(int target, int slot, int flags, int n, const int lanes[8], int w[4]) {
    unsigned long long lo = 0;
    for (int q = 0; q < 7; ++q) lo |= (unsigned long long)lanes[q] << (9 * q);
    w[0] = target;
    w[1] = own_pack_y(slot, flags, n, lanes[7]);
    w[2] = (int)(unsigned)(lo & 0xffffffffu);
    w[3] = (int)(unsigned)(lo >> 32);
}

HK_HD int own_slot(int y) { return (y & 1023) | ((y >> 18) & 1024); }
HK_HD int own_flags(int y) { return (y >> 10) & 15; }
HK_HD int own_n(int y) { return (y >> 14) & 15; }
HK_HD int own_lane(int y, int z, int w, int j) {
    const unsigned long long lo = (unsigned long long)(unsigned)z | ((unsigned long long)(unsigned)w << 32);
    return j < 7 ? (int)((lo >> (9 * j)) & 511) : (int)(((unsigned)y >> 18) & 511);
}

constexpr int kOwnTplMinEntries = 1 << 16;

HK_HD void own_pack_hdr(int toff, int count, int sofs, int tbase, int rbase, int h[4]) {
    h[0] = toff;
    h[1] = (int)((unsigned)count | (unsigned)sofs << 16);
    h[2] = tbase;
    h[3] = rbase;
}
HK_HD int own_hdr_count(int y) { return y & 0xffff; }
HK_HD int own_hdr_sofs(int y) { return (int)((unsigned)y >> 16); }
HK_HD int own_tpl_slot(int rel, int sofs, int P) {
    unsigned s = (unsigned)rel + (unsigned)sofs, t = s - (unsigned)P;
    s = t < s ? t : s;
    t = s - (unsigned)P;
    return (int)(t < s ? t : s);
}

}
```

### hakai-fem_amd/csrc/hakai_own_pass.hpp

```cpp
#pragma once
#include "hakai_elem_io.hpp"

namespace hk {


__device__ __forceinline__ void lds_barrier() {
    __builtin_amdgcn_fence(__ATOMIC_RELEASE, "workgroup", "local");
    __builtin_amdgcn_s_barrier();
    __builtin_amdgcn_fence(__ATOMIC_ACQUIRE, "workgroup", "local");
}

__device__ __forceinline__ int4 own_load(const ElemArgs& a, long long b) {
    const int o0 = a.own_off[b], o1 = a.own_off[b + 1];
    const int idx = o0 + (int)threadIdx.x;
    int4 en = a.own_list[idx < o1 ? idx : a.own_nop];
    en.y |= (o1 - o0 > kBlock) ? kOwnRound2 : 0;
    return en;
}

__device__ __forceinline__ int4 own_hdr_load(const ElemArgs& a, long long b) {
    typedef const int __attribute__((address_space(4))) * ConstInt;
    const ConstInt p = (ConstInt)(unsigned long long)(a.own_hdr + b);
    return make_int4(p[0], p[1], p[2], p[3]);
}

__device__ __forceinline__ int4 own_load_tpl(const ElemArgs& a, int4 h) {
    const int cnt = own_hdr_count(h.y);
    int4 en = a.own_list[(int)threadIdx.x < cnt ? h.x + (int)threadIdx.x : a.own_nop];
    en.y |= (cnt > kBlock) ? kOwnRound2 : 0;
    return en;
}

__device__ __forceinline__ int own_lane(int4 en, int j) { return own_lane(en.y, en.z, en.w, j); }

template <bool TPL>
__device__ __forceinline__ void own_entry(const ElemArgs& a, int4 en, int4 h, const double* s_fe, double* s_part) {
#pragma clang fp contract(off)
    const int flags = own_flags(en.y), n = own_n(en.y);
    int slot = own_slot(en.y);
    if (TPL) {
        if (!(flags & (kOwnExp | kOwnNop))) slot = own_tpl_slot(en.x, own_hdr_sofs(h.y), a.own_slots);
        en.x += (flags & kOwnExp) ? h.w : h.z;
    }
    double* dump = a.own_dump + 8 * (long long)blockIdx.x;
    double v[3];
    if (flags & (kOwnExp | kOwnNop)) {
#pragma unroll
        for (int j = 0; j < kOwnExpRows; ++j) {
            const int l = own_lane(en, j);
            double* dst = ((flags & kOwnExp) && j < n) ? a.own_rows + 3 * ((long long)en.x + (long long)j * slot) : dump;
#pragma unroll
            for (int c = 0; c < 3; ++c) dst[c] = s_fe[fe_at(l, c)];
        }
        return;
    }
#pragma unroll
    for (int c = 0; c < 3; ++c) v[c] = (flags & kOwnInit) ? 0.0 : s_part[3 * slot + c];
    for (int j = 0; j < n; ++j) {
        const int l = own_lane(en, j);
#pragma unroll
        for (int c = 0; c < 3; ++c) v[c] += s_fe[fe_at(l, c)];
    }
    if (!(flags & kOwnFin)) {
#pragma unroll
        for (int c = 0; c < 3; ++c) s_part[3 * slot + c] = v[c];
    }
    double* dst = (flags & kOwnFin) ? a.own_q + 3 * (long long)en.x : dump;
#pragma unroll
    for (int c = 0; c < 3; ++c) dst[c] = v[c];
}

#ifdef HK_DIAG_WAVE
struct PassClock {
    long long bar = 0, pass = 0, n = 0;
};
#define HK_DIAG_ARG , PassClock& dg
#define HK_DIAG_PASS , dg
#else
#define HK_DIAG_ARG
#define HK_DIAG_PASS
#endif

template <bool TPL>
__device__ __forceinline__ void own_pass(const ElemArgs& a, int4 en, int4 h, long long sb, const double* s_fe,
                                         double* s_part HK_DIAG_ARG) {
#ifdef HK_DIAG_WAVE
    const long long t0 = clock64();
#endif
    lds_barrier();
#ifdef HK_DIAG_WAVE
    const long long t1 = clock64();
#endif
    int o0, o1;
    if (TPL) {
        o0 = h.x;
        o1 = h.x + own_hdr_count(h.y);
    } else {
        o0 = a.own_off[sb];
        o1 = a.own_off[sb + 1];
    }
    if (o0 + (int)(threadIdx.x & ~63u) < o1) own_entry<TPL>(a, en, h, s_fe, s_part);
    if (en.y & kOwnRound2) {
        const int idx = o0 + kBlock + (int)threadIdx.x;
        if (o0 + kBlock + (int)(threadIdx.x & ~63u) < o1)
            own_entry<TPL>(a, a.own_list[idx < o1 ? idx : a.own_nop], h, s_fe, s_part);
    }
#ifdef HK_DIAG_WAVE
    const long long t2 = clock64();
    dg.bar += t1 - t0;
    dg.pass += t2 - t1;
    dg.n += 1;
#endif
}

}
```

### hakai-fem_amd/csrc/hakai_own_plan.cpp

```cpp
#include "hakai_own_plan.hpp"

#include <algorithm>
#include <cmath>
#include <cstring>
#include <unordered_map>
#include <utility>

#include "hakai_own_entry.hpp"

namespace hk {

static OwnSched own_contiguous(long long nb, long long G, int epb) {
    OwnSched sc;
    sc.epb = epb;
    sc.seq.resize(nb);
    for (long long b = 0; b < nb; ++b) sc.seq[b] = (int)b;
    sc.bstart.resize(G + 1);
    for (long long lb = 0; lb <= G; ++lb) sc.bstart[lb] = lb * nb / G;
    return sc;
}

static bool lattice_strides(const OwnInput& in, std::vector<int>& nx, std::vector<int>& L) {
    const long long nE = in.nE;
    nx.assign(nE, -1);
    L.assign(nE, -1);
    long long found = 0;
    for (long long e = 0; e < nE; ++e) {
        for (int k = 0; k < 8; ++k) {
            const int n = in.conn[8 * e + k];
            const int j0 = in.ptr[n];
            if (in.ptr[n + 1] - j0 != 8 || in.inc0[j0] / 8 != e) continue;
            long long q[8];
            for (int i = 0; i < 8; ++i) q[i] = in.inc0[j0 + i] / 8 - e;
            const long long a = q[2], l = q[4];
            if (q[1] == 1 && a > 1 && q[3] == a + 1 && l > a + 1 && q[5] == l + 1 && q[6] == l + a &&
                q[7] == l + a + 1 && l % a == 0 && l < (1LL << 30)) {
                nx[e] = (int)a;
                L[e] = (int)l;
                ++found;
                break;
            }
        }
    }
    if (found * 2 < nE) return false;
    long long first = -1;
    for (long long e = 0; e < nE; ++e)
        if (nx[e] > 0) {
            first = e;
            break;
        }
    for (long long e = 0; e < nE; ++e) {
        if (nx[e] > 0) continue;
        const long long src = e < first ? first : e - 1;
        nx[e] = nx[src];
        L[e] = L[src];
    }
    return true;
}

static bool own_banded(const OwnInput& in, long long G, const std::vector<int>& nx, const std::vector<int>& L,
                       int shrink, int epb, int slot_cap, OwnSched& sc) {
    const long long nb = in.nEp / epb, nE = in.nE;
    sc.epb = epb;
    std::vector<long long> rstart{0};
    for (long long x = 1; x < nE; ++x)
        if (nx[x] != nx[x - 1] || L[x] != L[x - 1]) rstart.push_back(x);
    rstart.push_back(nE);
    std::vector<long long> Rreg(rstart.size() - 1);
    for (size_t r = 0; r + 1 < rstart.size(); ++r) {
        const long long e0 = rstart[r], ne = rstart[r + 1] - e0;
        const long long rows = L[e0] / nx[e0], layers = std::max<long long>(1, ne / L[e0]);
        const double Gr = std::max(1.0, (double)G * (double)ne / (double)nE);
        const long long Rcap = (slot_cap - slot_cap / 16) / (nx[e0] + 1) - 1;
        const long long Ropt = (long long)std::llround(std::sqrt(1.5 * (double)layers * (double)rows / Gr));
        const long long Rwant = in.band_rows > 0 ? (long long)in.band_rows : std::max<long long>(Ropt, 1);
        Rreg[r] = std::max<long long>(1, std::min(Rcap, Rwant) - shrink);
    }
    std::vector<long long> key(nb);
    bool any_split = false;
    size_t region = 0;
    for (long long b = 0; b < nb; ++b) {
        const long long e = std::min(epb * b, nE - 1);
        while (e >= rstart[region + 1]) ++region;
        const long long rows = L[e] / nx[e];
        long long R = Rreg[region];
        if (R >= rows) R = rows;
        else any_split = true;
        const long long row = ((e - rstart[region]) % L[e]) / nx[e];
        key[b] = ((long long)region << 32) | (row / R);
    }
    if (!any_split) return false;
    std::vector<int> order(nb);
    for (long long b = 0; b < nb; ++b) order[b] = (int)b;
    std::stable_sort(order.begin(), order.end(), [&](int x, int y) { return key[x] < key[y]; });
    std::vector<std::pair<long long, long long>> bands;
    for (long long p = 0; p < nb;) {
        long long q = p;
        while (q < nb && key[order[q]] == key[order[p]]) ++q;
        bands.emplace_back(p, q);
        p = q;
    }
    const long long nbands = (long long)bands.size();
    if (nbands > G) return false;
    std::vector<long long> runs(nbands);
    std::vector<std::pair<double, long long>> rem;
    long long used = 0;
    for (long long i = 0; i < nbands; ++i) {
        const long long m = bands[i].second - bands[i].first;
        const double want = (double)G * (double)m / (double)nb;
        runs[i] = std::max<long long>(1, std::min<long long>(m, (long long)want));
        used += runs[i];
        rem.emplace_back(want - (double)runs[i], i);
    }
    std::sort(rem.begin(), rem.end(), [](const std::pair<double, long long>& x, const std::pair<double, long long>& y) {
        return x.first > y.first || (x.first == y.first && x.second < y.second);
    });
    for (size_t r = 0; used < G && r < rem.size(); ++r) {
        const long long i = rem[r].second;
        if (runs[i] < bands[i].second - bands[i].first) {
            ++runs[i];
            ++used;
        }
    }
    for (long long i = 0; used > G && i < nbands; ++i)
        while (runs[i] > 1 && used > G) {
            --runs[i];
            --used;
        }
    sc.seq = order;
    sc.bstart.assign(1, 0);
    for (long long i = 0; i < nbands; ++i) {
        const long long p = bands[i].first, m = bands[i].second - p;
        for (long long r = 1; r <= runs[i]; ++r) sc.bstart.push_back(p + r * m / runs[i]);
    }
    sc.banded = true;
    return true;
}

int OwnTplStore::add(const int* rel, int count) {
    unsigned long long h = 14695981039346656037ull ^ (unsigned)count;
    for (int q = 0; q < 4 * count; ++q) h = (h ^ (unsigned)rel[q]) * 1099511628211ull;
    std::vector<std::pair<int, int>>& cands = seen[h];
    for (const std::pair<int, int>& c : cands)
        if (c.second == count && (count == 0 || !std::memcmp(&tl[4 * (size_t)c.first], rel, sizeof(int) * 4 * (size_t)count)))
            return c.first;
    const int toff = (int)(tl.size() / 4);
    tl.insert(tl.end(), rel, rel + 4 * (size_t)count);
    cands.emplace_back(toff, count);
    ++distinct;
    return toff;
}

static bool own_plan(const OwnInput& in, const OwnSched& sc, int S, int slot_cap, OwnPlan& pl) {
    const int epb = sc.epb, bs = 8 * epb;
    const long long nb = in.nEp / epb, nN = in.nN;
    const long long G = (long long)sc.bstart.size() - 1;
    if (G <= 0 || in.max_inc > 8 || in.ptr.size() != (size_t)nN + 1) return false;
    pl.S = S;
    struct Ent { int target, slot, flags, n; int lanes[8]; int inc[4]; };
    std::vector<int> pos_of(nb), block_of(nb);
    std::vector<long long> sb_pos(nb);
    for (long long lb = 0; lb < G; ++lb)
        for (long long p = sc.bstart[lb]; p < sc.bstart[lb + 1]; ++p) {
            const int b = sc.seq[p];
            if (p > sc.bstart[lb] && b <= sc.seq[p - 1]) return false;
            pos_of[b] = (int)p;
            block_of[b] = (int)lb;
            sb_pos[b] = sc.bstart[lb] + (p - sc.bstart[lb]) / S * S;
        }
    std::vector<std::vector<Ent>> per(nb);
    std::vector<int> rp(nN + 1, 0);
    long long rows = 0;
    struct Seg { long long s0, s1; int node; std::vector<std::pair<long long, int>> refs; };
    std::vector<std::vector<Seg>> segs(G);
    auto batch_of = [&](int j) { return (long long)(in.inc0[j] / 8) / epb; };
    auto lane_of = [&](int j) {
        const long long e = in.inc0[j] / 8;
        const long long b = e / epb;
        return (int)(((pos_of[b] - sb_pos[b]) * epb + e % epb) * 8 + in.inc0[j] % 8);
    };
    std::vector<std::pair<long long, int>> exports;
    std::vector<char> all_rows(nN, 0);
    if (const std::vector<int>* dn = in.all_rows)
        for (int n : *dn) all_rows[n] = 1;
    for (long long n = 0; n < nN; ++n) {
        const int j0 = in.ptr[n], j1 = in.ptr[n + 1];
        if (j0 == j1) continue;
        if (all_rows[n]) {
            for (int j = j0; j < j1; ++j) exports.emplace_back(sb_pos[batch_of(j)], j);
            continue;
        }
        const int hb = block_of[batch_of(j0)];
        int j = j0;
        Seg sg;
        sg.s0 = -1;
        sg.node = (int)n;
        while (j < j1 && block_of[batch_of(j)] == hb) {
            const long long sb = sb_pos[batch_of(j)];
            Ent en{(int)n, 0, 0, 0, {0, 0, 0, 0, 0, 0, 0, 0}, {0, 0, 0, 0}};
            while (j < j1 && sb_pos[batch_of(j)] == sb) {
                if (en.n == 8) return false;
                en.lanes[en.n++] = lane_of(j);
                ++j;
            }
            if (sg.s0 < 0) {
                sg.s0 = sb;
                en.flags |= kOwnInit;
            }
            sg.s1 = sb;
            per[sb].push_back(en);
            sg.refs.emplace_back(sb, (int)per[sb].size() - 1);
        }
        per[sg.s1][sg.refs.back().second].flags |= kOwnFin;
        if (sg.s1 > sg.s0) segs[hb].push_back(std::move(sg));
        for (; j < j1; ++j) exports.emplace_back(sb_pos[batch_of(j)], j);
    }
    std::stable_sort(exports.begin(), exports.end(),
                     [](const std::pair<long long, int>& x, const std::pair<long long, int>& y) { return x.first < y.first; });
    std::vector<int> row_of_inc(in.inc0.size(), -1);
    for (size_t q = 0; q < exports.size();) {
        const long long sb = exports[q].first;
        Ent en{0, 0, kOwnExp, 0, {0, 0, 0, 0, 0, 0, 0, 0}, {0, 0, 0, 0}};
        while (q < exports.size() && exports[q].first == sb && en.n < kOwnExpRows) {
            const int j = exports[q].second;
            en.inc[en.n] = j;
            en.lanes[en.n++] = lane_of(j);
            ++q;
        }
        per[sb].push_back(en);
    }
    for (long long b = 0; b < nb; ++b) {
        std::vector<Ent>& v = per[b];
        for (size_t p = 0; p < v.size();) {
            if (!(v[p].flags & kOwnExp)) {
                ++p;
                continue;
            }
            size_t p1 = p;
            while (p1 < v.size() && (v[p1].flags & kOwnExp) && p1 / 64 == p / 64) ++p1;
            const int g = (int)(p1 - p);
            std::vector<std::pair<int, int>> cs;
            for (size_t i = p; i < p1; ++i)
                for (int k = 0; k < v[i].n; ++k) cs.emplace_back(v[i].inc[k], v[i].lanes[k]);
            const int m = (int)cs.size();
            for (int i = 0; i < g; ++i) {
                Ent& en = v[p + (size_t)i];
                en.target = (int)(rows + i);
                en.slot = g;
                en.n = 0;
                for (int q = i; q < m; q += g) {
                    en.inc[en.n] = cs[(size_t)q].first;
                    en.lanes[en.n++] = cs[(size_t)q].second;
                    row_of_inc[cs[(size_t)q].first] = (int)(rows + q);
                }
            }
            rows += m;
            p = p1;
        }
    }
    std::vector<int>& ridx = pl.ridx;
    ridx.clear();
    ridx.reserve(exports.size());
    for (long long n = 0; n < nN; ++n) {
        rp[n] = (int)ridx.size();
        for (int j = in.ptr[n]; j < in.ptr[n + 1]; ++j)
            if (row_of_inc[j] >= 0) ridx.push_back(row_of_inc[j]);
    }
    rp[nN] = (int)ridx.size();
    if (rows > (1LL << 31) - 1) return false;
    int max_slots = 1;
    for (long long lb = 0; lb < G; ++lb) {
        auto& v = segs[lb];
        std::sort(v.begin(), v.end(), [](const Seg& x, const Seg& y) { return x.s0 < y.s0; });
        std::vector<std::pair<long long, int>> busy;
        std::vector<int> free_slots;
        int next = 0;
        auto cmp = [](const std::pair<long long, int>& x, const std::pair<long long, int>& y) { return x.first > y.first; };
        for (auto& sg : v) {
            while (!busy.empty() && busy.front().first < sg.s0) {
                free_slots.push_back(busy.front().second);
                std::pop_heap(busy.begin(), busy.end(), cmp);
                busy.pop_back();
            }
            int slot;
            if (!free_slots.empty()) {
                slot = free_slots.back();
                free_slots.pop_back();
            } else {
                slot = next++;
            }
            if (slot >= slot_cap) return false;
            max_slots = std::max(max_slots, slot + 1);
            for (auto& r : sg.refs) per[r.first][r.second].slot = slot;
            busy.emplace_back(sg.s1, slot);
            std::push_heap(busy.begin(), busy.end(), cmp);
        }
    }
    std::vector<int>& off = pl.off;
    off.assign(nb + 1, 0);
    for (long long b = 0; b < nb; ++b) {
        if (per[b].size() > 2 * (size_t)bs) return false;
        pl.round2 += per[b].size() > (size_t)bs ? 1 : 0;
        off[b + 1] = off[b] + (int)per[b].size();
    }
    const long long ne = off[nb];
    std::vector<int>& list = pl.list;
    list.assign(4 * (size_t)(ne + 1), 0);
    for (long long b = 0; b < nb; ++b)
        for (size_t i = 0; i < per[b].size(); ++i) {
            const Ent& en = per[b][i];
            own_pack(en.target, en.slot, en.flags, en.n, en.lanes, &list[4 * ((size_t)off[b] + i)]);
        }
    const int no_lanes[8] = {0, 0, 0, 0, 0, 0, 0, 0};
    own_pack(0, 0, kOwnNop, 0, no_lanes, &list[4 * (size_t)ne]);
    pl.rp = std::move(rp);
    pl.rows = rows;
    pl.ne = ne;
    pl.max_slots = max_slots;
    pl.tpl = false;
    pl.P = 0;
    pl.hdr.clear();
    pl.tlist.clear();
    pl.stored = pl.templates = pl.passes = 0;
    if (!in.templates) return true;
    std::vector<int> tbase(nb, 0), rbase(nb, 0);
    long long max_rel = 0;
    for (long long b = 0; b < nb; ++b) {
        long long t0 = -1, t1 = -1, r0 = -1;
        for (const Ent& en : per[b]) {
            if (en.flags & kOwnExp) {
                r0 = r0 < 0 ? en.target : std::min<long long>(r0, en.target);
            } else {
                t0 = t0 < 0 ? en.target : std::min<long long>(t0, en.target);
                t1 = std::max<long long>(t1, en.target);
            }
        }
        tbase[b] = (int)std::max(t0, 0LL);
        rbase[b] = (int)std::max(r0, 0LL);
        max_rel = std::max(max_rel, t1 - t0);
    }
    std::vector<long long> until;
    auto valid = [&](int P) {
        for (long long lb = 0; lb < G; ++lb) {
            until.assign((size_t)P, -1);
            for (const Seg& sg : segs[lb]) {
                long long& u = until[(size_t)(sg.node % P)];
                if (u >= sg.s0) return false;
                u = sg.s1;
            }
        }
        return true;
    };
    int P = 0;
    {
        const long long least = std::max<long long>(max_slots, max_rel / 2 + 1);
        long long p2 = 1;
        while (p2 < least) p2 *= 2;
        for (; p2 <= slot_cap && !P; p2 *= 2)
            if (valid((int)p2)) P = (int)p2;
        for (long long p = slot_cap; p >= least && !P; --p)
            if (valid((int)p)) P = (int)p;
    }
    if (!P) return true;
    OwnTplStore store(pl.tlist);
    std::vector<int> rel;
    pl.hdr.assign(4 * (size_t)nb, 0);
    for (long long lb = 0; lb < G; ++lb)
        for (long long b = sc.bstart[lb]; b < sc.bstart[lb + 1]; b += S) {
            ++pl.passes;
            const int cnt = (int)per[b].size();
            rel.resize(4 * (size_t)cnt);
            for (int i = 0; i < cnt; ++i) {
                const Ent& en = per[b][(size_t)i];
                const bool ex = (en.flags & kOwnExp) != 0;
                own_pack(en.target - (ex ? rbase[b] : tbase[b]), ex ? en.slot : 0, en.flags, en.n, en.lanes, &rel[4 * (size_t)i]);
            }
            own_pack_hdr(store.add(rel.data(), cnt), cnt, tbase[b] % P, tbase[b], rbase[b], &pl.hdr[4 * (size_t)b]);
        }
    pl.templates = store.distinct;
    std::vector<int>& tl = pl.tlist;
    pl.stored = (long long)(tl.size() / 4);
    tl.resize(tl.size() + 4);
    own_pack(0, 0, kOwnNop, 0, no_lanes, &tl[4 * (size_t)pl.stored]);
    if (pl.ne >= kOwnTplMinEntries && 2 * (pl.stored + pl.passes) > pl.ne) {
        pl.hdr.clear();
        pl.tlist.clear();
        pl.stored = pl.templates = 0;
        return true;
    }
    pl.P = P;
    pl.tpl = true;
    return true;
}

bool own_choose(const OwnInput& in, long long G0, OwnSched& best_sc, OwnPlan& best, int only) {
    const int epb = 32;
    const long long nb = in.nEp / epb;
    auto cap_of = [&](int S) { return in.slot_cap[S - 1]; };
    const int cap = cap_of(2);
    bool have = false;
    auto consider = [&](const OwnSched& sc) {
        for (int S : {2, 1}) {
            if (in.pass_batches > 0 && S != in.pass_batches) continue;
            OwnPlan pl;
            if (!own_plan(in, sc, S, cap_of(S), pl)) continue;
            if (!have || pl.cost() < best.cost()) {
                best = std::move(pl);
                best_sc = sc;
                have = true;
            }
            return true;
        }
        return false;
    };
    if (only != 2) consider(own_contiguous(nb, G0, epb));
    if (only != 1) {
        std::vector<int> nx, L;
        if (lattice_strides(in, nx, L)) {
            OwnSched sc;
            for (int shrink : {0, 1, 2, 4})
                if (own_banded(in, G0, nx, L, shrink, epb, cap, sc) && consider(sc)) break;
        }
    }
    if (!have && only != 2 && 8 * G0 <= nb) consider(own_contiguous(nb, 8 * G0, epb));
    return have;
}

}
```

### hakai-fem_amd/csrc/hakai_own_plan.hpp

```cpp
#pragma once
#include <unordered_map>
#include <utility>
#include <vector>

namespace hk {

struct OwnSched {
    int epb = 32;
    std::vector<int> seq;
    std::vector<long long> bstart;
    bool banded = false;
};

struct OwnPlan {
    int S = 2;
    std::vector<int> off, list, rp, ridx;
    long long rows = 0, ne = 0;
    int max_slots = 1;
    long long round2 = 0;
    bool tpl = false;
    int P = 0;
    std::vector<int> hdr;
    std::vector<int> tlist;
    long long stored = 0;
    long long templates = 0;
    long long passes = 0;
    double cost() const { return 16.0 * (double)(tpl ? stored + passes : ne) + 52.0 * (double)rows; }
};

struct OwnTplStore {
    explicit OwnTplStore(std::vector<int>& store) : tl(store) {}
    int add(const int* rel, int count);
    long long distinct = 0;
private:
    std::vector<int>& tl;
    std::unordered_map<unsigned long long, std::vector<std::pair<int, int>>> seen;
};

struct OwnInput {
    long long nE, nN, nEp;
    const std::vector<int>& conn;
    const std::vector<int>& ptr;
    const std::vector<int>& inc0;
    int max_inc;
    int band_rows;
    int pass_batches;
    const std::vector<int>* all_rows;
    int slot_cap[2];
    int templates = 1;
};

bool own_choose(const OwnInput& in, long long G0, OwnSched& best_sc, OwnPlan& best, int only = 0);

}
```

### hakai-fem_amd/csrc/hakai_step.cpp

```cpp
#include <hip/hip_runtime.h>

#include <string>
#include <vector>

#include "../../include/hakai_hip.h"
#include "hakai_elem_history.hpp"
#include "hakai_history.hpp"
#include "hakai_internal.hpp"
#include "hakai_kernels.hpp"
#include "hakai_loads.hpp"

using hkc::fail;
using hkc::hip_fail;
using hkc::QSrc;

namespace hkc {
void graph_invalidate(hakai_ctx* c) {
    c->epoch++;
    c->tdev_next = -1;
}
void graph_free(hakai_ctx* c) {
    for (int g = 0; g < 2; ++g)
        for (int p = 0; p < 2; ++p)
            if (c->gr.exec[g][p]) {
                (void)hipGraphExecDestroy(c->gr.exec[g][p]);
                c->gr.exec[g][p] = nullptr;
                c->gr.epoch[g][p] = -1;
            }
}
}

enum { kPhaseA1 = 1, kPhaseRest = 2, kPhaseA2 = 4, kPhaseA3 = 8, kPhaseAll = 15 };
static int step_once(hakai_ctx* c, double t, double d_time, bool last, int phase = kPhaseAll) {
    hipStream_t s = c->stream;
    EventPair ep;
    if (c->contact) {
        const int part_bit[3] = {kPhaseA1, kPhaseA2, kPhaseA3};
        for (int part = 1; part <= 3; ++part) {
            if (!(phase & part_bit[part - 1]) || (part > 1 && !hkc::contact_multi(c))) continue;
            hkc::prof_begin(c, HAKAI_K_CONTACT, &ep);
            const int rc = hkc::contact_phase(c, part, t, d_time);
            hkc::prof_end(c, &ep);
            if (rc) return rc;
        }
    }
    if (!(phase & kPhaseRest)) return 0;
    const int par = c->sv.cur;
    const bool own = hkc::own_prepare(c);
    if (c->sv.q == QSrc::Own && !own) {
        if (int r = hkc::own_materialize(c)) return r;
    }
    hk::NodalArgs na = hkc::nodal_args(c, d_time);
    const hk::BCArgs ba = hkc::bc_args(c, t, d_time);
    const bool fuse_bc = c->bc.n > 0 && c->bc.d_of_node && c->fuse_bc && !c->comm &&
                         (c->nN <= kFuseBcMaxNodes || c->fuse_bc == 2);
    if (fuse_bc) {
        na.bc_of_node = c->bc.d_of_node;
        na.bc = ba;
    }
    int rc = 0;
    if (c->contact) {
        if (hkc::contact_multi(c)) {
            hkc::prof_begin(c, HAKAI_K_CONTACT_SUM, &ep);
            rc = hkc::contact_step_b(c);
            hkc::prof_end(c, &ep);
            if (rc) return rc;
        }
        na.fext = c->d_fext;
    }
    if (c->loads) {
        if ((rc = hkc::loads_step(c, t, d_time, na.fext))) return rc;
        na.fext = c->d_ftot;
    }
    rc = hkc::comm_pre_nodal(c);
    if (rc) return rc;
    if (c->hist && (rc = hkc::history_seed(c, na, s))) return rc;
    hkc::prof_begin(c, HAKAI_K_NODAL, &ep);
    HIPCHK(hk::launch_nodal(na, s));
    hkc::prof_end(c, &ep);
    hkc::CommFix fix;
    rc = hkc::comm_post_nodal(c, d_time, &fix);
    if (rc) return rc;
    if (c->bc.n > 0 && !fuse_bc) {
        hkc::prof_begin(c, HAKAI_K_BC, &ep);
        HIPCHK(hk::launch_bc(ba, s));
        hkc::prof_end(c, &ep);
    }
    if (c->hist && (rc = hkc::history_step(c, na, fix, t, c->gr.trd, s))) return rc;
    if (c->ehist && (rc = hkc::elem_history_step(c, t, c->gr.trd, s))) return rc;
    hk::ElemArgs ea = hkc::elem_args(c, 1 - par);
    ea.step_i = (int)t;
    if (own) hkc::own_elem_args(c, ea);
    if (c->gr.trd) {
        ea.t_rd = c->gr.trd;
        ea.t_wr = c->d_tstep + par;
    }
    hkc::prof_begin(c, HAKAI_K_ELEMENT, &ep);
    HIPCHK(hk::launch_element(ea, c->has_ductile, last, s));
    hkc::prof_end(c, &ep);
    c->sv.advance(own, last);
    c->own.steps += own ? 1 : 0;
    c->last_dt = d_time;
    rc = hkc::comm_post_element(c, (long long)t);
    if (rc) return rc;
    return hkc::contact_post_step(c);
}

static bool graph_eligible(const hakai_ctx* c, double t) {
    return c->graph && !c->comm && !c->prof && c->sv.q != QSrc::Buf && c->nE > 0 && hkc::contact_graph_ok(c, t) &&
           !hkc::history_needs_seed(c) && (c->sv.q == QSrc::Own) == hkc::own_wanted(c);
}

static int step_graph(hakai_ctx* c, double t, double d_time, int len) {
    hipStream_t s = c->stream;
    const int p0 = c->sv.cur;
    const int gi = len == 2 ? 1 : 0;
    hipGraphExec_t& ge = c->gr.exec[gi][p0];
    if (!c->d_tstep) HIPCHK(c->d_tstep.alloc(2));
    if (c->tdev_next != (long long)t) HIPCHK(hk::launch_set_step(c->d_tstep + (1 - p0), t - 1.0, s));
    if (ge && (c->gr.epoch[gi][p0] != c->epoch || c->gr.dt[gi][p0] != d_time || c->gr.len[gi][p0] != len)) {
        HIPCHK(hipStreamSynchronize(s));
        (void)hipGraphExecDestroy(ge);
        ge = nullptr;
    }
    if (!ge) {
        hipGraph_t g = nullptr;
        HIPCHK(hipStreamBeginCapture(s, hipStreamCaptureModeThreadLocal));
        int rc = 0;
        for (int k = 0; k < len && !rc; ++k) {
            c->gr.trd = c->d_tstep + (1 - c->sv.cur);
            rc = step_once(c, t + k, d_time, false);
        }
        c->gr.trd = nullptr;
        hipError_t e = hipStreamEndCapture(s, &g);
        if (rc) {
            if (g) (void)hipGraphDestroy(g);
            return rc;
        }
        if (e != hipSuccess) return hip_fail(e, "hipStreamEndCapture (step graph)");
        e = hipGraphInstantiate(&ge, g, nullptr, nullptr, 0);
        (void)hipGraphDestroy(g);
        if (e != hipSuccess) {
            ge = nullptr;
            return hip_fail(e, "hipGraphInstantiate (step graph)");
        }
        c->gr.epoch[gi][p0] = c->epoch;
        c->gr.dt[gi][p0] = d_time;
        c->gr.len[gi][p0] = len;
    } else {
        hkc::contact_graph_advance(c, t + len - 1);
        const bool own = c->sv.q == QSrc::Own;
        for (int k = 0; k < len; ++k) c->sv.advance(own, false);
        c->own.steps += own ? len : 0;
        c->last_dt = d_time;
    }
    HIPCHK(hipGraphLaunch(ge, s));
    c->tdev_next = (long long)t + len;
    c->graph_steps += len;
    return 0;
}

struct CallSnap {
    hkc::StepView sv;
    bool comm_pending = false;
    int comm_par = 0;
};
static CallSnap call_snap(const hakai_ctx* c) {
    CallSnap s;
    hkc::comm_pending_get(c, &s.comm_pending, &s.comm_par);
    s.sv = c->sv;
    return s;
}

static int finish_call(hakai_ctx* c, double t_first, int64_t n_steps, const CallSnap& s0) {
    const int rc = hkc::contact_check(c);
    if (rc && c->contact) {
        int pz[2] = {0, 0};
        HIPCHK(hipMemcpy(pz, c->d_poison, sizeof pz, hipMemcpyDeviceToHost));
        if (pz[0]) {
            c->poison_step = pz[1];
            const long long good = (long long)pz[1] - (long long)t_first;
            const bool rolled = good >= 0 && good <= n_steps;
            if (rolled) {
                c->sv.rollback(s0.sv, good);
                hkc::comm_rollback(c, good > 0, (long long)pz[1] - 1, s0.comm_pending, s0.comm_par);
            }
            hkc::graph_invalidate(c);
            hkc::contact_after_overflow(c, c->sv.steps_done);
            if (!rolled) (void)hkc::contact_exchange_retry(c);
            HIPCHK(hipMemset(c->d_poison, 0, 2 * sizeof(int)));
            const std::string msg = hakai_last_error();
            return fail(rc, "%s; step %d was not applied: the state is that after step %d", msg.c_str(), pz[1],
                        pz[1] - 1);
        }
    }
    return rc;
}

static int step_call(hakai_ctx* c, double t_first, int64_t n_steps, double d_time) {
    (void)hkc::own_prepare(c);
    const CallSnap s0 = call_snap(c);
    int64_t it = 0;
    while (it < n_steps) {
        const double t = t_first + (double)it;
        int rc;
        const int len = (c->graph > 2 && it + c->graph < n_steps) ? c->graph : 2;
        if (c->graph && it + len < n_steps && graph_eligible(c, t)) {
            rc = step_graph(c, t, d_time, len);
            it += len;
        } else {
            rc = step_once(c, t, d_time, it == n_steps - 1);
            c->tdev_next = -1;
            ++it;
        }
        if (rc) return rc;
    }
    return finish_call(c, t_first, n_steps, s0);
}

static int step_group_call(hakai_ctx** ctxs, int32_t n, double t_first, int64_t n_steps, double d_time) {
    std::vector<CallSnap> s0(n);
    for (int r = 0; r < n; ++r) {
        (void)hkc::own_prepare(ctxs[r]);
        s0[r] = call_snap(ctxs[r]);
    }
    const int phases[4] = {kPhaseA1, kPhaseA2, kPhaseA3, kPhaseRest};
    for (int64_t it = 0; it < n_steps; ++it) {
        const double t = t_first + (double)it;
        const bool last = it == n_steps - 1;
        for (int ph : phases)
            for (int r = 0; r < n; ++r) {
                if (ctxs[0]->group_serial == 2) HIPCHK(hk::launch_hold(96, ctxs[r]->stream));
                if (int rc = step_once(ctxs[r], t, d_time, last, ph)) return rc;
                if (ph == kPhaseRest) ctxs[r]->tdev_next = -1;
                if (ctxs[0]->group_serial) HIPCHK(hipStreamSynchronize(ctxs[r]->stream));
            }
    }
    int first = 0;
    for (int r = 0; r < n; ++r) {
        const int rc = finish_call(ctxs[r], t_first, n_steps, s0[r]);
        if (rc && !first) first = rc;
    }
    return first;
}

static constexpr int kExchangeRetries = 8;

extern "C" {

int hakai_step(hakai_ctx* c, double t_first, int64_t n_steps, double d_time) {
    if (!c) return fail(HAKAI_ERR_ARG, "null");
    if (!c->model_ok || !c->state_ok) return fail(HAKAI_ERR_STATE, "step before upload_model/reset_state");
    if (n_steps < 0 || !(d_time > 0)) return fail(HAKAI_ERR_ARG, "step: n_steps=%lld d_time=%g", (long long)n_steps, d_time);
    if (n_steps > 1 && hkc::comm_is_local(c))
        return fail(HAKAI_ERR_ARG, "step: an in-process group is stepped one step per call, rank by rank");
    if (hkc::comm_is_local(c) && hkc::contact_multi(c) && hkc::comm_size(c) > 1)
        return fail(HAKAI_ERR_STATE, "step: rank %d of an in-process group with multi-GPU contact is stepped by "
                    "hakai_step_group only", hkc::comm_rank(c));
    HIPCHK(hipSetDevice(c->device));
    for (int attempt = 0;; ++attempt) {
        const int rc = step_call(c, t_first, n_steps, d_time);
        if (!rc || attempt >= kExchangeRetries || !hkc::contact_exchange_retry(c)) return rc;
        ++c->exchange_retries;
        n_steps -= (int64_t)(c->poison_step - (long long)t_first);
        t_first = (double)c->poison_step;
    }
}

int hakai_step_group(hakai_ctx** ctxs, int32_t n, double t_first, int64_t n_steps, double d_time) {
    if (!ctxs || n <= 0) return fail(HAKAI_ERR_ARG, "step_group: no contexts");
    if (n_steps < 0 || !(d_time > 0)) return fail(HAKAI_ERR_ARG, "step_group: n_steps=%lld d_time=%g",
                                                  (long long)n_steps, d_time);
    for (int r = 0; r < n; ++r) {
        hakai_ctx* c = ctxs[r];
        if (!c) return fail(HAKAI_ERR_ARG, "step_group: null context %d", r);
        if (!c->model_ok || !c->state_ok) return fail(HAKAI_ERR_STATE, "step_group: rank %d has no model/state", r);
        if (n > 1 && (!c->comm || hkc::comm_rank(c) != r || hkc::comm_size(c) != n ||
                      hkc::comm_peer_ctx(c, r) != c))
            return fail(HAKAI_ERR_ARG, "step_group: context %d is not rank %d of an in-process group of %d", r, r, n);
        hkc::graph_invalidate(c);
    }
    HIPCHK(hipSetDevice(ctxs[0]->device));
    for (int attempt = 0;; ++attempt) {
        const int rc = step_group_call(ctxs, n, t_first, n_steps, d_time);
        if (!rc || attempt >= kExchangeRetries) return rc;
        bool retry = true;
        for (int r = 0; r < n; ++r) retry = hkc::contact_exchange_retry(ctxs[r]) && retry;
        if (!retry) return rc;
        const long long p = ctxs[0]->poison_step;
        for (int r = 1; r < n; ++r)
            if (ctxs[r]->poison_step != p)
                return fail(rc, "step_group: ranks disagree on the poisoned step (rank 0: %lld, rank %d: %lld)", p, r,
                            ctxs[r]->poison_step);
        for (int r = 0; r < n; ++r) ++ctxs[r]->exchange_retries;
        n_steps -= (int64_t)(p - (long long)t_first);
        t_first = (double)p;
    }
}

int hakai_graph_steps(hakai_ctx* c, int64_t* n) {
    if (!c || !n) return fail(HAKAI_ERR_ARG, "null");
    *n = c->graph_steps;
    return 0;
}

}
```

### hakai-fem_amd/csrc/hakai_step_view.hpp

```cpp
#pragma once

namespace hkc {

enum class QSrc { Fe, Buf, Own };

struct StepView {
    int cur = 0;
    long long steps_done = 0;
    bool fe_ok = true, triax_ok = true;
    QSrc q = QSrc::Fe;

    void advance(bool own, bool last) {
        cur = 1 - cur;
        q = own ? QSrc::Own : QSrc::Fe;
        fe_ok = !own || last;
        triax_ok = last;
        steps_done++;
    }
    void rollback(const StepView& s0, long long good) {
        cur = (good & 1) ? 1 - s0.cur : s0.cur;
        steps_done = s0.steps_done + good;
        if (good == 0) {
            fe_ok = s0.fe_ok;
            triax_ok = s0.triax_ok;
            q = s0.q;
        } else {
            fe_ok = q != QSrc::Own;
            triax_ok = false;
        }
    }
    void restart(bool keep_cur) {
        if (!keep_cur) {
            cur = 0;
            q = QSrc::Fe;
        }
        own_dropped();
        fe_ok = triax_ok = true;
        steps_done = 0;
    }
    void q_uploaded() { q = QSrc::Buf; }
    void own_dropped() { if (q == QSrc::Own) q = QSrc::Fe; }
};

}
```

Baseline: 2654.

## Fold nodal displacement update into owner-assembly pass of fused element kernel

For nodes whose final owner-assembly entry lands in a block, the element kernel now computes the explicit nodal displacement update directly and writes it to the next displacement buffer. The separate nodal kernel then processes only the remaining residual nodes through an index list. This removes one full pass of nodal reads and writes (mass, u, force, Q) for most nodes. The cost is extra state tracking across steps, a doubled set of cached step graphs, and the restriction that the path only applies without contact, loads, comm or history.

```diff
diff --git a/hakai-fem_amd/csrc/hakai_capi.cpp b/hakai-fem_amd/csrc/hakai_capi.cpp
--- a/hakai-fem_amd/csrc/hakai_capi.cpp
+++ b/hakai-fem_amd/csrc/hakai_capi.cpp
@@ -761,7 +761,8 @@
     if (!std::strcmp(key, "graph_steps")) *value = c->graph_steps;
     else if (!std::strcmp(key, "device_buffers")) *value = hkc::g_dev_live.load();
     else if (!std::strcmp(key, "exchange_retries")) *value = c->exchange_retries;
-    else if (!std::strncmp(key, "own_", 4) || !std::strncmp(key, "conn_", 5)) return hkc::own_stat(c, key, value);
+    else if (!std::strncmp(key, "own_", 4) || !std::strncmp(key, "conn_", 5) || !std::strncmp(key, "fold_", 5))
+        return hkc::own_stat(c, key, value);
     else return fail(HAKAI_ERR_ARG, "unknown stat '%s'", key);
     return 0;
 }
diff --git a/hakai-fem_amd/csrc/hakai_elem_fused.hpp b/hakai-fem_amd/csrc/hakai_elem_fused.hpp
--- a/hakai-fem_amd/csrc/hakai_elem_fused.hpp
+++ b/hakai-fem_amd/csrc/hakai_elem_fused.hpp
@@ -5,9 +5,14 @@
 namespace hk {
 
 
-template <bool DO_DELETE, bool STORE_TRIAX, bool ANY_PLASTIC, bool WITH_VOL, int NT = 0, bool OWN = false>
+struct NoPreWb {
+    __device__ __forceinline__ void operator()() const {}
+};
+template <bool DO_DELETE, bool STORE_TRIAX, bool ANY_PLASTIC, bool WITH_VOL, int NT = 0, bool OWN = false,
+          class PreWb = NoPreWb>
 __device__ __forceinline__ void elem_step(const ElemArgs& a, const DevMat* __restrict__ mats, long long e, int k,
-                                          double* nd8, const ElemIn& in, double* sfe = nullptr) {
+                                          double* nd8, const ElemIn& in, double* sfe = nullptr,
+                                          PreWb pre_wb = PreWb()) {
     const DevMat* M = mats + in.mt;
     const bool active = in.fl == 1;
     const int npp = M->npp;
@@ -170,6 +175,7 @@
     fk[1] += S * bb1;
     fk[2] += S * bb2;
     if (WITH_VOL) a.vol[e] = V;
+    pre_wb();
     elem_writeback<DO_DELETE, STORE_TRIAX, ANY_PLASTIC, NT, false, OWN>(a, e, k, in, active, kill, fk, fin, eps, eqp,
                                                                          ys, tri, sfe);
 }
diff --git a/hakai-fem_amd/csrc/hakai_element.hip b/hakai-fem_amd/csrc/hakai_element.hip
--- a/hakai-fem_amd/csrc/hakai_element.hip
+++ b/hakai-fem_amd/csrc/hakai_element.hip
@@ -50,7 +50,7 @@
 #endif
 
 template <bool DO_DELETE, bool STORE_TRIAX, bool ANY_PLASTIC, bool LDS_MATS, int NT, bool EXACT, int OS = 0,
-          bool TPL = false, bool CT = false>
+          bool TPL = false, bool CT = false, bool FOLD = false>
 __global__ __launch_bounds__(kBlock, 2) void k_element_pipe(ElemArgs a) {
     constexpr bool OWN = OS > 0;
     constexpr int kOwnFe = OS * kEPB * kFeStride;
@@ -110,6 +110,7 @@
     load_stage_a<EXACT, CT>(a, elem_of(0), k, cur);
     load_stage_a<EXACT, CT>(a, elem_of(1), k, nxt);
     static_assert(!(CT && EXACT), "connectivity templates: fused kernel only");
+    static_assert(!FOLD || (OS > 0 && TPL && !EXACT && !STORE_TRIAX), "nodal fold: fused template-form owner assembly");
     int rec_nn = 0;
     if (CT) {
         const int r0 = conn_rec(a, elem_of(0)), r1 = conn_rec(a, elem_of(1));
@@ -141,6 +142,7 @@
         if (!EXACT) load_stage_b<ANY_PLASTIC, NT>(a, elem_of(i + 1), k, nxt);
         if (OWN) ent_nxt = TPL ? own_load_tpl(a, hdr_nxt) : own_load(a, sb_of(i + 1));
         double* sfe = s_fe + ((i / S) & 1) * kOwnFe + (i % S) * (kEPB * kFeStride);
+        FoldIn fin;
         if (EXACT) {
 #ifdef HK_DIAG_PHASE
             pc.last = clock64();
@@ -151,11 +153,18 @@
             elem_step_exact<DO_DELETE, STORE_TRIAX, ANY_PLASTIC, false, NT, OWN>(a, mats, elem_of(i), k, nd8, xb, s_pus,
                                                                                  cur, sfe HK_PH_PASS);
         }
-        else
+        else if (FOLD) {
+            const bool pass_next = (i + 1) % S == 0 || i + 1 == count;
+            const unsigned ft = fold_node(ent_cur, hdr_cur);
+            elem_step<DO_DELETE, STORE_TRIAX, ANY_PLASTIC, false, NT, OWN>(a, mats, elem_of(i), k, nd8, cur, sfe, [&]() {
+                if (pass_next) fold_load(a, ft, fin);
+            });
+        } else
             elem_step<DO_DELETE, STORE_TRIAX, ANY_PLASTIC, false, NT, OWN>(a, mats, elem_of(i), k, nd8, cur, sfe);
         if (OWN) {
             if ((i + 1) % S == 0 || i + 1 == count)
-                own_pass<TPL>(a, ent_cur, hdr_cur, sb_of(i), s_fe + ((i / S) & 1) * kOwnFe, s_part HK_DIAG_PASS);
+                own_pass<TPL, FOLD>(a, ent_cur, hdr_cur, sb_of(i), s_fe + ((i / S) & 1) * kOwnFe, s_part,
+                                    &fin HK_DIAG_PASS);
             ent_cur = ent_nxt;
             if (TPL) {
                 hdr_cur = hdr_nxt;
@@ -218,8 +227,8 @@
            ...);
 }
 
-constexpr bool pipe_exists(bool lds_mats, bool exact, int os, bool tpl, bool ct) {
-    return (os > 0 ? lds_mats : !tpl) && (!ct || (!exact && tpl));
+constexpr bool pipe_exists(bool lds_mats, bool exact, int os, bool tpl, bool ct, bool store_triax, bool fold) {
+    return (os > 0 ? lds_mats : !tpl) && (!ct || (!exact && tpl)) && (!fold || (!exact && tpl && !store_triax));
 }
 
 static void launch_pipe(const ElemArgs& a, bool do_delete, bool store_triax, unsigned grid, hipStream_t s) {
@@ -227,15 +236,16 @@
     const bool lds = os > 0 || a.nmat <= kMaxLdsMats;
     const bool tpl = os > 0 && a.own_hdr;
     const bool ct = !a.exact && tpl && a.conn_rec;
+    const bool fold = a.fold_out != nullptr;
     const size_t dyn = (os > 0 ? 24 * (size_t)a.own_slots : 0) + (lds ? sizeof(DevMat) * (size_t)a.nmat : 0);
     with_consts(
-        [&](auto DD, auto ST, auto AP, auto LDS, auto NT, auto EX, auto OS, auto TPL, auto CT) {
-            if constexpr (pipe_exists(LDS(), EX(), OS(), TPL(), CT()))
-                hipLaunchKernelGGL((k_element_pipe<DD(), ST(), AP(), LDS(), NT(), EX(), OS(), TPL(), CT()>), dim3(grid),
-                                   dim3(kBlock), dyn, s, a);
+        [&](auto DD, auto ST, auto AP, auto LDS, auto NT, auto EX, auto OS, auto TPL, auto CT, auto FOLD) {
+            if constexpr (pipe_exists(LDS(), EX(), OS(), TPL(), CT(), ST(), FOLD()))
+                hipLaunchKernelGGL((k_element_pipe<DD(), ST(), AP(), LDS(), NT(), EX(), OS(), TPL(), CT(), FOLD()>),
+                                   dim3(grid), dim3(kBlock), dyn, s, a);
         },
         sel(do_delete), sel(store_triax), sel(a.any_plastic != 0), sel(lds), sel<0, 3>(a.gp_nt ? 3 : 0),
-        sel(a.exact != 0), sel<0, 1, 2>(os), sel(tpl), sel(ct));
+        sel(a.exact != 0), sel<0, 1, 2>(os), sel(tpl), sel(ct), sel(fold));
 }
 
 static void launch_batch(const ElemArgs& a, bool do_delete, bool store_triax, unsigned grid, hipStream_t s) {
@@ -260,7 +270,10 @@
             return hipErrorInvalidValue;
         if (a.own_grid <= 0 || a.own_grid > nb) return hipErrorInvalidValue;
         if (a.conn_rec && (a.conn_bits < 0 || a.conn_bits > 31)) return hipErrorInvalidValue;
+        if (a.fold_out && (a.exact || !a.own_hdr || store_triax || !a.mass || !(a.dt > 0))) return hipErrorInvalidValue;
         launch_pipe(a, do_delete, store_triax, (unsigned)a.own_grid, s);
+    } else if (a.fold_out) {
+        return hipErrorInvalidValue;
     } else if (a.pipe_blocks > 0 && !a.vol) {
         launch_pipe(a, do_delete, store_triax, (unsigned)std::min<long long>(nb, a.pipe_blocks), s);
     } else {
diff --git a/hakai-fem_amd/csrc/hakai_internal.hpp b/hakai-fem_amd/csrc/hakai_internal.hpp
--- a/hakai-fem_amd/csrc/hakai_internal.hpp
+++ b/hakai-fem_amd/csrc/hakai_internal.hpp
@@ -100,10 +100,11 @@
     hkc::DevBuf<double> d_tstep;
     struct StepGraphs {
         const double* trd = nullptr;
-        hipGraphExec_t exec[2][2] = {{nullptr, nullptr}, {nullptr, nullptr}};
-        double dt[2][2] = {{0.0, 0.0}, {0.0, 0.0}};
-        long long epoch[2][2] = {{-1, -1}, {-1, -1}};
-        int len[2][2] = {{0, 0}, {0, 0}};
+        hipGraphExec_t exec[2][4] = {{nullptr, nullptr, nullptr, nullptr}, {nullptr, nullptr, nullptr, nullptr}};
+        double dt[2][4] = {{0.0, 0.0, 0.0, 0.0}, {0.0, 0.0, 0.0, 0.0}};
+        long long epoch[2][4] = {{-1, -1, -1, -1}, {-1, -1, -1, -1}};
+        int len[2][4] = {{0, 0, 0, 0}, {0, 0, 0, 0}};
+        bool fold[2][4] = {{false, false, false, false}, {false, false, false, false}};
     } gr;
     long long epoch = 0;
     long long tdev_next = -1;
diff --git a/hakai-fem_amd/csrc/hakai_kernels.hpp b/hakai-fem_amd/csrc/hakai_kernels.hpp
--- a/hakai-fem_amd/csrc/hakai_kernels.hpp
+++ b/hakai-fem_amd/csrc/hakai_kernels.hpp
@@ -56,6 +56,9 @@
     double* own_q;
     double* own_rows;
     double* own_dump;
+    double* fold_out;
+    const double* mass;
+    double dt;
 };
 
 struct BCArgs {
@@ -93,6 +96,8 @@
     const int* own_rp;
     const int* own_ridx;
     const double* own_rows;
+    const int* res = nullptr;
+    long long n_res = -1;
 };
 
 
diff --git a/hakai-fem_amd/csrc/hakai_nodal.hip b/hakai-fem_amd/csrc/hakai_nodal.hip
--- a/hakai-fem_amd/csrc/hakai_nodal.hip
+++ b/hakai-fem_amd/csrc/hakai_nodal.hip
@@ -1,6 +1,7 @@
 #include <hip/hip_runtime.h>
 
 #include "hakai_kernels.hpp"
+#include "hakai_nodal_update.hpp"
 
 namespace hk {
 
@@ -24,10 +25,6 @@
     return a.val[i] * amp;
 }
 
-struct NodeIn {
-    double m, uc[3], up[3], f[3];
-};
-
 template <bool FEXT>
 __device__ __forceinline__ void nodal_load(const NodalArgs& a, long long n, NodeIn& in) {
     in.m = a.mass[n];
@@ -43,17 +40,12 @@
 __device__ __forceinline__ void nodal_update(const NodalArgs& a, long long n, const NodeIn& in, double Q0, double Q1,
                                              double Q2) {
 #pragma clang fp contract(off)
-    const double m = in.m;
-    const double dt = a.dt;
-    const double dC = 0.0 * m;
-    const double mdt2 = m / (dt * dt);
-    const double inv = 1.0 / (mdt2 + dC / 2.0 / dt);
+    const NodalCoef kc = nodal_coef(in.m, a.dt);
     const double Q[3] = {Q0, Q1, Q2};
     const int b0 = BCF ? a.bc_of_node[n] : -1;
 #pragma unroll
     for (int c = 0; c < 3; ++c) {
-        const double up = in.up[c];
-        double v = inv * (in.f[c] - Q[c] + mdt2 * (2.0 * in.uc[c] - up) + dC / 2.0 / dt * up);
+        double v = nodal_disp(kc, in.uc[c], in.up[c], in.f[c], Q[c]);
         if (BCF) {
             const long long dc = 3 * n + c;
             for (int j = b0; j >= 0 && j < a.bc.n && a.bc.dof[j] <= dc; ++j)
@@ -68,8 +60,13 @@
 #pragma clang fp contract(off)
     if (poisoned(a.poison)) return;
     const unsigned lb = xcd_remap_rev(blockIdx.x, gridDim.x);
-    const long long n = (long long)lb * kBlock + threadIdx.x;
-    if (n >= a.nN) return;
+    long long n = (long long)lb * kBlock + threadIdx.x;
+    if (MODE == 4) {
+        if (n >= a.n_res) return;
+        n = a.res[n];
+    } else if (n >= a.nN) {
+        return;
+    }
     NodeIn in;
     nodal_load<FEXT>(a, n, in);
     double Q0 = 0.0, Q1 = 0.0, Q2 = 0.0;
@@ -77,7 +74,7 @@
         Q0 = a.qbuf[3 * n + 0];
         Q1 = a.qbuf[3 * n + 1];
         Q2 = a.qbuf[3 * n + 2];
-    } else if (MODE == 3) {
+    } else if (MODE == 3 || MODE == 4) {
         Q0 = a.own_q[3 * n + 0];
         Q1 = a.own_q[3 * n + 1];
         Q2 = a.own_q[3 * n + 2];
@@ -132,6 +129,13 @@
 
 hipError_t launch_nodal(const NodalArgs& a, hipStream_t s) {
     if (a.nN <= 0) return hipSuccess;
+    if (a.n_res >= 0) {
+        if (!a.own_q || a.qbuf || a.fext || a.bc_of_node || (a.n_res > 0 && !a.res)) return hipErrorInvalidValue;
+        if (a.n_res == 0) return hipSuccess;
+        hipLaunchKernelGGL((k_nodal<4, false, false>), dim3((unsigned)((a.n_res + kBlock - 1) / kBlock)), dim3(kBlock), 0,
+                           s, a);
+        return hipGetLastError();
+    }
     const unsigned grid = (unsigned)((a.nN + kBlock - 1) / kBlock);
     if (a.bc_of_node) {
         if (a.fext)
diff --git a/hakai-fem_amd/csrc/hakai_nodal_update.hpp b/hakai-fem_amd/csrc/hakai_nodal_update.hpp
--- /dev/null
+++ b/hakai-fem_amd/csrc/hakai_nodal_update.hpp
@@ -0,0 +1,29 @@
+#pragma once
+#include <hip/hip_runtime.h>
+
+namespace hk {
+
+struct NodeIn {
+    double m, uc[3], up[3], f[3];
+};
+
+struct NodalCoef {
+    double mdt2, inv, dCh;
+};
+
+__device__ __forceinline__ NodalCoef nodal_coef(double m, double dt) {
+#pragma clang fp contract(off)
+    NodalCoef k;
+    const double dC = 0.0 * m;
+    k.mdt2 = m / (dt * dt);
+    k.dCh = dC / 2.0 / dt;
+    k.inv = 1.0 / (k.mdt2 + k.dCh);
+    return k;
+}
+
+__device__ __forceinline__ double nodal_disp(const NodalCoef& k, double uc, double up, double f, double Q) {
+#pragma clang fp contract(off)
+    return k.inv * (f - Q + k.mdt2 * (2.0 * uc - up) + k.dCh * up);
+}
+
+}
diff --git a/hakai-fem_amd/csrc/hakai_own.cpp b/hakai-fem_amd/csrc/hakai_own.cpp
--- a/hakai-fem_amd/csrc/hakai_own.cpp
+++ b/hakai-fem_amd/csrc/hakai_own.cpp
@@ -38,7 +38,7 @@
                 : l.d_off.upload(pl.off, s) || l.d_list.upload(pl.list, s)) ||
         l.d_seq.upload(sc.seq, s) || l.d_bstart.upload(bst, s) || l.d_rp.upload(pl.rp, s) || l.d_ridx.upload(pl.ridx, s) ||
         l.d_q.alloc(3 * (size_t)nN) || l.d_rows.alloc(3 * (size_t)std::max(pl.rows, 1LL)) ||
-        l.d_dump.alloc(8 * (size_t)G) ||
+        l.d_dump.alloc(8 * (size_t)G) || (pl.tpl && !pl.res.empty() && l.d_res.upload(pl.res, s)) ||
         hipMemsetAsync(l.d_q, 0, 3 * (size_t)nN * sizeof(double), s) ||
         hipStreamSynchronize(s)) {
         own_free(c);
@@ -54,6 +54,8 @@
     l.s = pl.S;
     l.round2 = pl.round2;
     l.banded = sc.banded ? 1 : 0;
+    l.n_res = (long long)pl.res.size();
+    l.fold_nodes = pl.tpl ? pl.fold_nodes : 0;
     return true;
 }
 
@@ -88,7 +90,7 @@
                               c->own.band_rows, c->own.pass_batches, comm_dn_nodes(c),
                               {hk::own_slot_cap(c->elem_exact != 0, 1, c->nmat),
                                hk::own_slot_cap(c->elem_exact != 0, 2, c->nmat)},
-                              c->own.templates};
+                              c->own.templates, c->own.fold};
         hk::OwnSched sc;
         hk::OwnPlan pl;
         if (!(hk::own_choose(in, G0, sc, pl) && own_upload(c, sc, pl))) {
@@ -124,8 +126,31 @@
     }
 }
 
+bool own_fold_ok(const hakai_ctx* c) {
+    const Own::Lists& l = c->own.l;
+    return c->own.fold && !c->elem_exact && l.d_hdr.get() && l.fold_nodes > 0 && !c->contact && !c->loads && !c->comm &&
+           !c->hist && !c->ehist;
+}
+
+void own_fold_elem_args(const hakai_ctx* c, double d_time, hk::ElemArgs& ea) {
+    ea.fold_out = const_cast<double*>(ea.u_pre);
+    ea.mass = c->d_mass;
+    ea.dt = d_time;
+}
+
+void own_fold_nodal_args(const hakai_ctx* c, hk::NodalArgs& na) {
+    na.res = c->own.l.d_res;
+    na.n_res = c->own.l.n_res;
+}
+
 int own_tuning(hakai_ctx* c, const char* key, long long value) {
     Own& o = c->own;
+    if (!std::strcmp(key, "own_fold")) {
+        if (value < 0 || value > 1) return fail(HAKAI_ERR_ARG, "own_fold must be 0 or 1");
+        if (o.fold != (int)value) o.for_g0 = -1;
+        o.fold = (int)value;
+        return 0;
+    }
     if (!std::strcmp(key, "own_assembly")) {
         if (value < 0 || value > 2) return fail(HAKAI_ERR_ARG, "own_assembly must be 0, 1 or 2");
         o.assembly = (int)value;
@@ -176,6 +201,8 @@
     else if (!std::strcmp(key, "own_slots")) *value = built ? l.slots : 0;
     else if (!std::strcmp(key, "own_banded")) *value = built ? l.banded : 0;
     else if (!std::strcmp(key, "own_grid")) *value = built ? l.built_g : 0;
+    else if (!std::strcmp(key, "fold_nodes")) *value = built ? l.fold_nodes : 0;
+    else if (!std::strcmp(key, "fold_steps")) *value = c->own.fold_steps;
     else if (!std::strcmp(key, "conn_patterns")) *value = conn_in_use(c) ? c->conn_P : 0;
     else if (!std::strcmp(key, "conn_bytes")) *value = conn_in_use(c) ? c->conn_bytes : 32 * c->nEp;
     else return fail(HAKAI_ERR_ARG, "unknown stat '%s'", key);
diff --git a/hakai-fem_amd/csrc/hakai_own.hpp b/hakai-fem_amd/csrc/hakai_own.hpp
--- a/hakai-fem_amd/csrc/hakai_own.hpp
+++ b/hakai-fem_amd/csrc/hakai_own.hpp
@@ -11,6 +11,8 @@
     int band_rows = 0;
     int pass_batches = 0;
     int templates = 1;
+    int fold = 1;
+    long long fold_steps = 0;
     long long for_g0 = -1;
     long long steps = 0;
     struct Lists {
@@ -33,6 +35,8 @@
         DevBuf<double> d_dump;
         long long rows = 0, entries = 0;
         int s = 2;
+        DevBuf<int> d_res;
+        long long n_res = 0, fold_nodes = 0;
     } l;
 };
 
@@ -50,6 +54,9 @@
 bool own_wanted(const hakai_ctx* c);
 int own_materialize(hakai_ctx* c);
 void own_elem_args(const hakai_ctx* c, hk::ElemArgs& ea);
+bool own_fold_ok(const hakai_ctx* c);
+void own_fold_elem_args(const hakai_ctx* c, double d_time, hk::ElemArgs& ea);
+void own_fold_nodal_args(const hakai_ctx* c, hk::NodalArgs& na);
 int own_tuning(hakai_ctx* c, const char* key, long long value);
 int own_stat(const hakai_ctx* c, const char* key, int64_t* value);
 
diff --git a/hakai-fem_amd/csrc/hakai_own_entry.hpp b/hakai-fem_amd/csrc/hakai_own_entry.hpp
--- a/hakai-fem_amd/csrc/hakai_own_entry.hpp
+++ b/hakai-fem_amd/csrc/hakai_own_entry.hpp
@@ -18,6 +18,9 @@
                  ((unsigned)slot & 1024u) << 18);
 }
 static_assert((own_pack_y(kOwnSlotsMax - 1, 15, 15, 511) & kOwnRound2) == 0, "kOwnRound2 overlaps a packed field");
+constexpr int kOwnFold = 1 << 29;
+static_assert((own_pack_y(kOwnSlotsMax - 1, 15, 15, 511) & kOwnFold) == 0 && kOwnFold != kOwnRound2,
+              "kOwnFold overlaps a packed field");
 
 HK_HD void own_pack(int target, int slot, int flags, int n, const int lanes[8], int w[4]) {
     unsigned long long lo = 0;
diff --git a/hakai-fem_amd/csrc/hakai_own_pass.hpp b/hakai-fem_amd/csrc/hakai_own_pass.hpp
--- a/hakai-fem_amd/csrc/hakai_own_pass.hpp
+++ b/hakai-fem_amd/csrc/hakai_own_pass.hpp
@@ -1,5 +1,6 @@
 #pragma once
 #include "hakai_elem_io.hpp"
+#include "hakai_nodal_update.hpp"
 
 namespace hk {
 
@@ -33,8 +34,24 @@
 
 __device__ __forceinline__ int own_lane(int4 en, int j) { return own_lane(en.y, en.z, en.w, j); }
 
-template <bool TPL>
-__device__ __forceinline__ void own_entry(const ElemArgs& a, int4 en, int4 h, const double* s_fe, double* s_part) {
+struct FoldIn {
+    double m, uc[3], up[3];
+};
+__device__ __forceinline__ unsigned fold_node(int4 en, int4 h) {
+    return (own_flags(en.y) & (kOwnExp | kOwnNop)) ? 0u : (unsigned)(en.x + h.z);
+}
+__device__ __forceinline__ void fold_load(const ElemArgs& a, unsigned t, FoldIn& fi) {
+    fi.m = *at32(a.mass, 8u * t);
+#pragma unroll
+    for (int c = 0; c < 3; ++c) {
+        fi.uc[c] = at32(a.u, 24u * t)[c];
+        fi.up[c] = at32(a.u_pre, 24u * t)[c];
+    }
+}
+
+template <bool TPL, bool FOLD = false>
+__device__ __forceinline__ void own_entry(const ElemArgs& a, int4 en, int4 h, const double* s_fe, double* s_part,
+                                          const FoldIn* fi = nullptr) {
 #pragma clang fp contract(off)
     const int flags = own_flags(en.y), n = own_n(en.y);
     int slot = own_slot(en.y);
@@ -65,9 +82,18 @@
 #pragma unroll
         for (int c = 0; c < 3; ++c) s_part[3 * slot + c] = v[c];
     }
-    double* dst = (flags & kOwnFin) ? a.own_q + 3 * (long long)en.x : dump;
+    const bool fold = FOLD && (en.y & kOwnFold);
+    double* dst = ((flags & kOwnFin) && !fold) ? a.own_q + 3 * (long long)en.x : dump;
 #pragma unroll
     for (int c = 0; c < 3; ++c) dst[c] = v[c];
+    if (FOLD) {
+        FoldIn f = *fi;
+        asm volatile("" : "+v"(f.m), "+v"(f.uc[0]), "+v"(f.uc[1]), "+v"(f.uc[2]), "+v"(f.up[0]), "+v"(f.up[1]), "+v"(f.up[2]));
+        const NodalCoef kc = nodal_coef(f.m, a.dt);
+        double* du = fold ? a.fold_out + 3 * (long long)en.x : dump + 3;
+#pragma unroll
+        for (int c = 0; c < 3; ++c) du[c] = nodal_disp(kc, f.uc[c], f.up[c], 0.0, v[c]);
+    }
 }
 
 #ifdef HK_DIAG_WAVE
@@ -81,9 +107,9 @@
 #define HK_DIAG_PASS
 #endif
 
-template <bool TPL>
+template <bool TPL, bool FOLD = false>
 __device__ __forceinline__ void own_pass(const ElemArgs& a, int4 en, int4 h, long long sb, const double* s_fe,
-                                         double* s_part HK_DIAG_ARG) {
+                                         double* s_part, const FoldIn* fi HK_DIAG_ARG) {
 #ifdef HK_DIAG_WAVE
     const long long t0 = clock64();
 #endif
@@ -99,7 +125,7 @@
         o0 = a.own_off[sb];
         o1 = a.own_off[sb + 1];
     }
-    if (o0 + (int)(threadIdx.x & ~63u) < o1) own_entry<TPL>(a, en, h, s_fe, s_part);
+    if (o0 + (int)(threadIdx.x & ~63u) < o1) own_entry<TPL, FOLD>(a, en, h, s_fe, s_part, fi);
     if (en.y & kOwnRound2) {
         const int idx = o0 + kBlock + (int)threadIdx.x;
         if (o0 + kBlock + (int)(threadIdx.x & ~63u) < o1)
diff --git a/hakai-fem_amd/csrc/hakai_own_plan.cpp b/hakai-fem_amd/csrc/hakai_own_plan.cpp
--- a/hakai-fem_amd/csrc/hakai_own_plan.cpp
+++ b/hakai-fem_amd/csrc/hakai_own_plan.cpp
@@ -157,7 +157,7 @@
     const long long G = (long long)sc.bstart.size() - 1;
     if (G <= 0 || in.max_inc > 8 || in.ptr.size() != (size_t)nN + 1) return false;
     pl.S = S;
-    struct Ent { int target, slot, flags, n; int lanes[8]; int inc[4]; };
+    struct Ent { int target, slot, flags, n; int lanes[8]; int inc[4]; int fold; };
     std::vector<int> pos_of(nb), block_of(nb);
     std::vector<long long> sb_pos(nb);
     for (long long lb = 0; lb < G; ++lb)
@@ -197,7 +197,7 @@
         sg.node = (int)n;
         while (j < j1 && block_of[batch_of(j)] == hb) {
             const long long sb = sb_pos[batch_of(j)];
-            Ent en{(int)n, 0, 0, 0, {0, 0, 0, 0, 0, 0, 0, 0}, {0, 0, 0, 0}};
+            Ent en{(int)n, 0, 0, 0, {0, 0, 0, 0, 0, 0, 0, 0}, {0, 0, 0, 0}, 0};
             while (j < j1 && sb_pos[batch_of(j)] == sb) {
                 if (en.n == 8) return false;
                 en.lanes[en.n++] = lane_of(j);
@@ -212,6 +212,7 @@
             sg.refs.emplace_back(sb, (int)per[sb].size() - 1);
         }
         per[sg.s1][sg.refs.back().second].flags |= kOwnFin;
+        if (j == j1 && sg.refs.back().second < bs) per[sg.s1][sg.refs.back().second].fold = 1;
         if (sg.s1 > sg.s0) segs[hb].push_back(std::move(sg));
         for (; j < j1; ++j) exports.emplace_back(sb_pos[batch_of(j)], j);
     }
@@ -220,7 +221,7 @@
     std::vector<int> row_of_inc(in.inc0.size(), -1);
     for (size_t q = 0; q < exports.size();) {
         const long long sb = exports[q].first;
-        Ent en{0, 0, kOwnExp, 0, {0, 0, 0, 0, 0, 0, 0, 0}, {0, 0, 0, 0}};
+        Ent en{0, 0, kOwnExp, 0, {0, 0, 0, 0, 0, 0, 0, 0}, {0, 0, 0, 0}, 0};
         while (q < exports.size() && exports[q].first == sb && en.n < kOwnExpRows) {
             const int j = exports[q].second;
             en.inc[en.n] = j;
@@ -322,6 +323,8 @@
     pl.hdr.clear();
     pl.tlist.clear();
     pl.stored = pl.templates = pl.passes = 0;
+    pl.fold_nodes = 0;
+    pl.res.clear();
     if (!in.templates) return true;
     std::vector<int> tbase(nb, 0), rbase(nb, 0);
     long long max_rel = 0;
@@ -374,6 +377,7 @@
                 const Ent& en = per[b][(size_t)i];
                 const bool ex = (en.flags & kOwnExp) != 0;
                 own_pack(en.target - (ex ? rbase[b] : tbase[b]), ex ? en.slot : 0, en.flags, en.n, en.lanes, &rel[4 * (size_t)i]);
+                if (in.fold && en.fold) rel[4 * (size_t)i + 1] |= kOwnFold;
             }
             own_pack_hdr(store.add(rel.data(), cnt), cnt, tbase[b] % P, tbase[b], rbase[b], &pl.hdr[4 * (size_t)b]);
         }
@@ -390,6 +394,16 @@
     }
     pl.P = P;
     pl.tpl = true;
+    if (in.fold) {
+        std::vector<char> folded(nN, 0);
+        for (long long b = 0; b < nb; ++b)
+            for (const Ent& en : per[b])
+                if (en.fold) folded[en.target] = 1;
+        for (long long n = 0; n < nN; ++n) {
+            if (folded[n]) ++pl.fold_nodes;
+            else pl.res.push_back((int)n);
+        }
+    }
     return true;
 }
 
diff --git a/hakai-fem_amd/csrc/hakai_own_plan.hpp b/hakai-fem_amd/csrc/hakai_own_plan.hpp
--- a/hakai-fem_amd/csrc/hakai_own_plan.hpp
+++ b/hakai-fem_amd/csrc/hakai_own_plan.hpp
@@ -25,6 +25,8 @@
     long long stored = 0;
     long long templates = 0;
     long long passes = 0;
+    long long fold_nodes = 0;
+    std::vector<int> res;
     double cost() const { return 16.0 * (double)(tpl ? stored + passes : ne) + 52.0 * (double)rows; }
 };
 
@@ -48,6 +50,7 @@
     const std::vector<int>* all_rows;
     int slot_cap[2];
     int templates = 1;
+    int fold = 1;
 };
 
 bool own_choose(const OwnInput& in, long long G0, OwnSched& best_sc, OwnPlan& best, int only = 0);
diff --git a/hakai-fem_amd/csrc/hakai_step.cpp b/hakai-fem_amd/csrc/hakai_step.cpp
--- a/hakai-fem_amd/csrc/hakai_step.cpp
+++ b/hakai-fem_amd/csrc/hakai_step.cpp
@@ -21,7 +21,7 @@
 }
 void graph_free(hakai_ctx* c) {
     for (int g = 0; g < 2; ++g)
-        for (int p = 0; p < 2; ++p)
+        for (int p = 0; p < 4; ++p)
             if (c->gr.exec[g][p]) {
                 (void)hipGraphExecDestroy(c->gr.exec[g][p]);
                 c->gr.exec[g][p] = nullptr;
@@ -52,7 +52,11 @@
     }
     hk::NodalArgs na = hkc::nodal_args(c, d_time);
     const hk::BCArgs ba = hkc::bc_args(c, t, d_time);
-    const bool fuse_bc = c->bc.n > 0 && c->bc.d_of_node && c->fuse_bc && !c->comm &&
+    const bool folded = c->sv.folded;
+    if (folded && !(own && c->sv.q == QSrc::Own && !c->contact && !c->loads && !c->comm && !c->hist))
+        return fail(HAKAI_ERR_STATE, "step: the previous element step folded a nodal update this step cannot complete");
+    if (folded) hkc::own_fold_nodal_args(c, na);
+    const bool fuse_bc = c->bc.n > 0 && c->bc.d_of_node && c->fuse_bc && !c->comm && !folded &&
                          (c->nN <= kFuseBcMaxNodes || c->fuse_bc == 2);
     if (fuse_bc) {
         na.bc_of_node = c->bc.d_of_node;
@@ -91,6 +95,8 @@
     hk::ElemArgs ea = hkc::elem_args(c, 1 - par);
     ea.step_i = (int)t;
     if (own) hkc::own_elem_args(c, ea);
+    const bool fold = own && !last && hkc::own_fold_ok(c);
+    if (fold) hkc::own_fold_elem_args(c, d_time, ea);
     if (c->gr.trd) {
         ea.t_rd = c->gr.trd;
         ea.t_wr = c->d_tstep + par;
@@ -98,8 +104,9 @@
     hkc::prof_begin(c, HAKAI_K_ELEMENT, &ep);
     HIPCHK(hk::launch_element(ea, c->has_ductile, last, s));
     hkc::prof_end(c, &ep);
-    c->sv.advance(own, last);
+    c->sv.advance(own, last, fold);
     c->own.steps += own ? 1 : 0;
+    c->own.fold_steps += fold ? 1 : 0;
     c->last_dt = d_time;
     rc = hkc::comm_post_element(c, (long long)t);
     if (rc) return rc;
@@ -115,10 +122,11 @@
     hipStream_t s = c->stream;
     const int p0 = c->sv.cur;
     const int gi = len == 2 ? 1 : 0;
-    hipGraphExec_t& ge = c->gr.exec[gi][p0];
+    const int ps = p0 + (c->sv.folded ? 2 : 0);
+    hipGraphExec_t& ge = c->gr.exec[gi][ps];
     if (!c->d_tstep) HIPCHK(c->d_tstep.alloc(2));
     if (c->tdev_next != (long long)t) HIPCHK(hk::launch_set_step(c->d_tstep + (1 - p0), t - 1.0, s));
-    if (ge && (c->gr.epoch[gi][p0] != c->epoch || c->gr.dt[gi][p0] != d_time || c->gr.len[gi][p0] != len)) {
+    if (ge && (c->gr.epoch[gi][ps] != c->epoch || c->gr.dt[gi][ps] != d_time || c->gr.len[gi][ps] != len)) {
         HIPCHK(hipStreamSynchronize(s));
         (void)hipGraphExecDestroy(ge);
         ge = nullptr;
@@ -144,14 +152,17 @@
             ge = nullptr;
             return hip_fail(e, "hipGraphInstantiate (step graph)");
         }
-        c->gr.epoch[gi][p0] = c->epoch;
-        c->gr.dt[gi][p0] = d_time;
-        c->gr.len[gi][p0] = len;
+        c->gr.epoch[gi][ps] = c->epoch;
+        c->gr.dt[gi][ps] = d_time;
+        c->gr.len[gi][ps] = len;
+        c->gr.fold[gi][ps] = c->sv.folded;
     } else {
         hkc::contact_graph_advance(c, t + len - 1);
         const bool own = c->sv.q == QSrc::Own;
-        for (int k = 0; k < len; ++k) c->sv.advance(own, false);
+        const bool fold = c->gr.fold[gi][ps];
+        for (int k = 0; k < len; ++k) c->sv.advance(own, false, fold);
         c->own.steps += own ? len : 0;
+        c->own.fold_steps += fold ? len : 0;
         c->last_dt = d_time;
     }
     HIPCHK(hipGraphLaunch(ge, s));
diff --git a/hakai-fem_amd/csrc/hakai_step_view.hpp b/hakai-fem_amd/csrc/hakai_step_view.hpp
--- a/hakai-fem_amd/csrc/hakai_step_view.hpp
+++ b/hakai-fem_amd/csrc/hakai_step_view.hpp
@@ -9,9 +9,11 @@
     long long steps_done = 0;
     bool fe_ok = true, triax_ok = true;
     QSrc q = QSrc::Fe;
+    bool folded = false;
 
-    void advance(bool own, bool last) {
+    void advance(bool own, bool last, bool fold = false) {
         cur = 1 - cur;
+        folded = fold;
         q = own ? QSrc::Own : QSrc::Fe;
         fe_ok = !own || last;
         triax_ok = last;
@@ -20,6 +22,7 @@
     void rollback(const StepView& s0, long long good) {
         cur = (good & 1) ? 1 - s0.cur : s0.cur;
         steps_done = s0.steps_done + good;
+        folded = good == 0 ? s0.folded : false;
         if (good == 0) {
             fe_ok = s0.fe_ok;
             triax_ok = s0.triax_ok;
@@ -35,6 +38,7 @@
             q = QSrc::Fe;
         }
         own_dropped();
+        folded = false;
         fe_ok = triax_ok = true;
         steps_done = 0;
     }
```

Result: no change. 2653, median of 2 (-0.0%).
